# JuliaQuantumControl/QuOptimalControl.jl

Measured on AMD Instinct MI355X. Metric: GRAPE gradient-evals/sec, higher is better.
Workload: dtype f64; 1 GPU; C3: UnitaryGate 4x4, K=4, N=500 slices, ensemble E=1024 (one GPU, 1024 members/GPU), T=2.0; step = host->host grape_eval; parallelism=single GPU

## Files before the change

### quoptimalcontrol.jl_amd/csrc/grape_api.cpp

```cpp
#include "../../include/grape_hip.h"

#include <hip/hip_runtime.h>
#include <rccl/rccl.h>

#include <dlfcn.h>
#include <fcntl.h>
#include <time.h>
#include <unistd.h>

#include <algorithm>
#include <cmath>
#include <complex>
#include <cstdio>
#include <cstdlib>
#include <cstring>
#include <limits>
#include <atomic>
#include <condition_variable>
#include <mutex>
#include <thread>
#include <new>
#include <utility>
#include <string>
#include <vector>
// ... 104 lines not shown
    int32_t *d_any_sp_i = nullptr;
    double2 *d_any_sp_c = nullptr;
    size_t any_sp_i_bytes = 0, any_sp_c_bytes = 0, any_sp_nnz = 0, any_sp_ntouch = 0;
    bool ctrl_scaled = false;
    double *d_ctrl_scale = nullptr;
    size_t act_var_bytes = 0;
    double *d_act_bn = nullptr;
    double2 *d_act_bs = nullptr;
    int32_t *d_act_bo = nullptr;
    size_t states_bytes = 0;
    int tp_C = 0, tp_S = 0;
    double2 *d_tp_q = nullptr, *d_tp_r = nullptr, *d_tp_m = nullptr;
    double *d_tp_z = nullptr;
    double2 *d_tp_vec = nullptr;
    size_t tp_cap[6] = {0, 0, 0, 0, 0, 0};
    int tp_G = 0, tp_g = 0;
    double2 *d_tp_a = nullptr;
    bool direct_publish = true;
    bool pen_on = false;
    std::vector<double> pen_w;
    double *d_pen_w = nullptr;
    int rc_terms = 0;
    double2 *d_rc_R = nullptr;
    double *d_rc_rho = nullptr;
    double2 *d_rc_xs = nullptr;
    double *d_rc_rows = nullptr;
    size_t rc_xs_bytes = 0, rc_rows_bytes = 0;
    int rc_mode = 0;
    bool obs_on = false;
    int obs_n = 0, obs_per_member = 0;
    bool obs_want_y = false, obs_want_xf = false;
    double2 *d_obs_O = nullptr;
    double2 *d_obs_y = nullptr;
    double2 *d_obs_xf = nullptr;
    size_t obs_O_bytes = 0, obs_y_bytes = 0, obs_xf_bytes = 0;
    bool vjp_on = false;
    int vjp_n = 0, vjp_per_member = 0;
    bool vjp_has_y = false, vjp_has_x = false;
    double2 *d_vjp_O = nullptr;
    double2 *d_vjp_ybar = nullptr;
    double2 *d_vjp_xbar = nullptr;
    double *d_vjp_part = nullptr;
    double *d_vjp_g = nullptr;
    double *d_vjp_out = nullptr;
    size_t vjp_O_bytes = 0, vjp_ybar_bytes = 0, vjp_xbar_bytes = 0, vjp_part_bytes = 0, vjp_g_bytes = 0, vjp_out_bytes = 0;
    const double2 *obs_O_call = nullptr, *vjp_O_call = nullptr, *vjp_ybar_call = nullptr, *vjp_xbar_call = nullptr;
    double2 *obs_y_call = nullptr, *obs_xf_call = nullptr;
    double *vjp_G_call = nullptr;
    int obs_staged = 0, vjp_staged = 0;
    bool jvp_on = false;
    int jvp_n = 0, jvp_per_member = 0;
    bool jvp_has_y = false, jvp_has_x = false;
    double2 *d_jvp_O = nullptr;
    double *d_jvp_xdot = nullptr;
    double *d_jvp_xphys = nullptr;
    double2 *d_jvp_ydot = nullptr;
    double2 *d_jvp_xf = nullptr;
    size_t jvp_O_bytes = 0, jvp_xdot_bytes = 0, jvp_xphys_bytes = 0, jvp_ydot_bytes = 0, jvp_xf_bytes = 0;
    const double2 *jvp_O_call = nullptr;
    const double *jvp_xdot_call = nullptr;
    double2 *jvp_ydot_call = nullptr, *jvp_xf_call = nullptr;
    int jvp_ndir = 0, jvp_multi = 0;
    int lds_cap = 0;
    bool traj_valid = false;
    int traj_mode = 0;
    double2 *d_traj_w = nullptr;
    double *d_traj_x = nullptr;
    size_t traj_w_bytes = 0, traj_x_bytes = 0;
    int basis_M = 0;
    int basis_nb = 1;
    double *d_basis_phi = nullptr;
    double *d_basis_x0 = nullptr;
    bool bounds_on = false;
    double *d_bounds = nullptr;
    double *d_slope = nullptr;
    double risk_beta = 0.0;
    double *d_risk_rows = nullptr;
    double *d_risk_p = nullptr;
    size_t risk_rows_bytes = 0, risk_p_bytes = 0;
    int risk_slot = 0;
    bool risk_evaluated = false;
    std::vector<double> h_wts;
    bool pair_ah_env = true;
    bool mf_publish = true;
    unsigned long long seq = 0;
    std::string kernel_log;
    int x_upload = 1;
    double *d_x_bar = nullptr;
    hipStream_t stream = nullptr;
    bool ops_set = false, evaluated = false;
    bool unitary = false;
    bool herm_states = false;
    std::vector<hipEvent_t> ev;
    std::vector<char> ev_has_mid;
    std::vector<float> smp_total, smp_first;
    uint64_t ev_issued = 0, ev_folded = 0;
    uint64_t launches = 0;
    double ev_total_ms = 0.0;
    int64_t ev_count = 0;
    hipEvent_t ev_dev = nullptr;
    bool dev_pending = false;
    ncclComm_t comm = nullptr;
    int comm_rank = 0, comm_size = 1;
    bool is_group = false;
    std::vector<grape_ctx *> sub;
    std::vector<int> sub_lo;
    struct GroupWorker *worker = nullptr;
    double group_tm[5] = {0, 0, 0, 0, 0};
    uint64_t group_tm_n = 0;
    double timeout_s = 600.0;
    double eval_ema_s = 0.0;
    mutable std::string err;
};

static constexpr size_t kEventRing = 256;

static thread_local std::string *g_kernel_log = nullptr;
struct KernelLogScope {
    explicit KernelLogScope(std::string *log, bool append = false) { g_kernel_log = log; if (log && !append) log->clear(); }
    ~KernelLogScope() { g_kernel_log = nullptr; }
};
namespace grape {
void log_kernel(const char *expr)
{
    std::string *log = g_kernel_log;
    if (!log || !expr) return;
    while (*expr == '(' || *expr == ' ') ++expr;
    const char *end = expr;
    while (*end && *end != '<' && *end != ')' && *end != ' ') ++end;
    if (!log->empty()) log->push_back(';');
    log->append(expr, (size_t)(end - expr));
}
}

static thread_local std::string g_create_err = "";

static int fail(const grape_ctx *ctx, int code, const std::string &msg)
{
    if (ctx) ctx->err = msg; else g_create_err = msg;
    return code;
}

#define HIP_TRY(ctx, call)                                                                     \
    do {                                                                                       \
        hipError_t e__ = (call);                                                               \
        if (e__ != hipSuccess)                                                                 \
            return fail(ctx, e__ == hipErrorOutOfMemory ? GRAPE_ERR_ALLOC : GRAPE_ERR_HIP,     \
                        std::string(#call) + ": " + hipGetErrorString(e__));                   \
    } while (0)

static double now_s()
{
    timespec t;
    clock_gettime(CLOCK_MONOTONIC, &t);
    return (double)t.tv_sec + 1e-9 * (double)t.tv_nsec;
}

static const grape_ctx *lead_of(const grape_ctx *c) { return c->is_group ? c->sub[0] : c; }
static grape_ctx *lead_of(grape_ctx *c) { return c->is_group ? c->sub[0] : c; }

template <class T>
static int grow(grape_ctx *c, T **ptr, size_t *cap, size_t want, const char *who, const char *what)
{
    if (want <= *cap) return GRAPE_OK;
    (void)hipFree(*ptr);
    *ptr = nullptr;
// ... 433 lines not shown
    if (const char *ev = std::getenv("GRAPE_MPB")) {
        const int v = std::atoi(ev);
        if (c->family == 0 && v >= 1 && v * W <= wmax) c->MPB = v;
    }
    if (c->MPB > E) c->MPB = E;
    bool xg_in_lds = true;
    if (c->family == 0) {
        const size_t cap = 150 * 1024;
        auto lds_need = [&](int mpb, bool in_lds) {
            return c->pair ? grape::sweep_pair_lds_bytes(cfg->n, mpb, c->LT, S, cfg->n_controls, in_lds)
                           : grape::sweep_small_lds_bytes(cfg->n, mpb, c->LT, S, cfg->n_controls, in_lds);
        };
        while (c->MPB > 1 && lds_need(c->MPB, true) > cap)
            c->MPB /= 2;
        xg_in_lds = lds_need(c->MPB, true) <= cap;
    }
    c->NB = (E + c->MPB - 1) / c->MPB;
    c->ksplit = grape::reduce_ksplit(E);

    const size_t nn = (size_t)cfg->n * cfg->n, K = cfg->n_controls;
    const size_t Q = KN(c) + 1;
    c->ws_unit = c->family == 0 ? (size_t)S * nn * c->CH : (c->family == 1 ? (size_t)N * c->TSZ : (size_t)N * nn);
    const size_t ops_elems = c->family != 1 ? (size_t)E * (K + 3) * nn : (size_t)c->EU * (2 * K + 3) * c->TSZ;
    const bool exact = cfg->gradient == GRAPE_GRADIENT_EXACT;
    const bool keepl = (cfg->flags & GRAPE_FLAG_KEEP_COSTATES) != 0 || exact;
    {
        size_t free_b = 0, total_b = 0;
        if (hipMemGetInfo(&free_b, &total_b) != hipSuccess || free_b == 0) {
            hipDeviceProp_t pr{};
            free_b = hipGetDeviceProperties(&pr, c->device) == hipSuccess ? pr.totalGlobalMem : ~(size_t)0 >> 1;
        }
        const size_t rest = 2 * (sizeof(double2) * ops_elems + sizeof(double) * (size_t)E * Q * c->B) + ((size_t)64 << 20);
        c->ws_budget = free_b > rest ? (size_t)(0.9 * (double)(free_b - rest)) : 0;
        if (const char *ev = std::getenv("GRAPE_MAX_WORKSPACE_BYTES")) c->ws_budget = (size_t)std::strtoull(ev, nullptr, 10);
        if (const char *ev = std::getenv("GRAPE_TEST_FAIL_REPLAN")) c->test_fail_replan = std::atoi(ev);
        if (!plan_chunk(c, 1 + (keepl ? 1 : 0))) {
            const std::string msg = "grape_create: not even " + std::to_string(c->family == 0 ? c->MPB : 2) +
                                    " members' workspace fits the budget of " + std::to_string(c->ws_budget) + " bytes";
            delete c;
            return fail(nullptr, GRAPE_ERR_ALLOC, msg);
        }
    }

    auto alloc = [&](void **p, size_t bytes) -> hipError_t {
        c->bytes += bytes;
        return hipMalloc(p, bytes);
    };
    hipError_t e = hipSuccess;
    if (e == hipSuccess) e = alloc((void **)&c->d_ops, sizeof(double2) * ops_elems);
    if (e == hipSuccess) e = alloc((void **)&c->d_wts, sizeof(double) * E);
    const size_t Bn = (size_t)c->B;
    if (e == hipSuccess) e = alloc((void **)&c->d_x, sizeof(double) * KN(c) * Bn);
    if (e == hipSuccess) e = alloc((void **)&c->d_fg, sizeof(double) * Q * Bn);
    if (e == hipSuccess) e = alloc((void **)&c->d_props, sizeof(double2) * c->ws_elems * ws_batch(c));
    if (e == hipSuccess && keepl) e = alloc((void **)&c->d_costates, sizeof(double2) * c->ws_elems * ws_batch(c));
    if (e == hipSuccess && exact && c->family == 0) e = alloc((void **)&c->d_zphi, sizeof(double) * 2 * E * Bn);
    const bool want_rows = c->family != 0 || (cfg->flags & GRAPE_FLAG_MEMBER_RESULTS) || exact;
    if (e == hipSuccess && want_rows) e = alloc((void **)&c->d_member_out, sizeof(double) * E * Q * Bn);
    if (e == hipSuccess) e = alloc((void **)&c->d_partial, sizeof(double) * c->ksplit * Q);
    if (e == hipSuccess && c->family == 0) e = alloc((void **)&c->d_block_out, sizeof(double) * c->NB * Q * Bn);
    if (e == hipSuccess && c->family == 0 && !xg_in_lds)
        e = alloc((void **)&c->d_xg_scratch,
                  sizeof(double) * Bn * c->NB * ((size_t)c->MPB * c->CH * ((size_t)S * K + 1) + c->MPB));
    if (e == hipSuccess && (cfg->flags & GRAPE_FLAG_PHASE_STAMPS)) {
        const size_t sb = sizeof(unsigned long long) * Bn * E * W * grape::kStampSlots;
        e = alloc((void **)&c->d_stamps, sb);
        if (e == hipSuccess) e = hipMemset(c->d_stamps, 0, sb);
    }
    const unsigned hflags = hipHostMallocMapped | hipHostMallocCoherent | hipHostMallocPortable;
    if (e == hipSuccess) e = hipHostMalloc((void **)&c->h_stage, sizeof(double) * Q * Bn, hflags);
    if (e == hipSuccess) e = hipHostGetDevicePointer((void **)&c->d_h_stage, c->h_stage, 0);
    if (e == hipSuccess) e = hipHostMalloc((void **)&c->h_fg, sizeof(double) * Q * Bn, hflags);
    if (e == hipSuccess) e = hipHostGetDevicePointer((void **)&c->d_h_fg, c->h_fg, 0);
    if (e == hipSuccess) e = hipHostMalloc((void **)&c->h_flag, 64 + sizeof(unsigned long long) * grape::kMaxMflags, hflags);
    if (e == hipSuccess) e = hipHostGetDevicePointer((void **)&c->d_h_flag, c->h_flag, 0);
    if (e == hipSuccess) { std::memset(c->h_flag, 0, 64 + sizeof(unsigned long long) * grape::kMaxMflags); e = alloc((void **)&c->d_done_counter, 64); }
    if (e == hipSuccess) e = hipMemset(c->d_done_counter, 0, 64);
    {
        const char *dp = std::getenv("GRAPE_DIRECT_PUBLISH");
        c->direct_publish = !(dp && dp[0] == '0');
        c->mf_publish = !env_off("GRAPE_MF_PUBLISH");
        c->pair_ah_env = !env_off("GRAPE_PAIR_AH");
        c->pair_image_env = !env_off("GRAPE_PAIR_IMAGE");
    }
    {
        const char *xu = std::getenv("GRAPE_X_UPLOAD");
        int mode = 2;
        if (xu) mode = !std::strcmp(xu, "memcpy") ? 0 : (!std::strcmp(xu, "kernel") ? 1 : 2);
        int large_bar = 0;
        if (mode == 2 && e == hipSuccess &&
            (hipDeviceGetAttribute(&large_bar, hipDeviceAttributeIsLargeBar, dev) != hipSuccess || !large_bar))
            mode = 1;
        if (mode == 2 && e == hipSuccess) {
            void *p = nullptr;
            if (hipExtMallocWithFlags(&p, sizeof(double) * KN(c) * Bn, hipDeviceMallocFinegrained) == hipSuccess && p) {
                const int fd = open("/dev/zero", O_RDONLY);
                const bool ok = fd >= 0 && read(fd, p, 64) == 64;
                if (fd >= 0) close(fd);
                if (ok) {
                    c->d_x_bar = (double *)p;
                    c->bytes += sizeof(double) * KN(c) * Bn;
                } else {
                    (void)hipFree(p);
                    mode = 1;
                }
            } else {
                (void)hipGetLastError();
                mode = 1;
            }
        }
        c->x_upload = mode;
        if (std::getenv("GRAPE_DEBUG"))
            std::fprintf(stderr, "[grape] x upload mode %d (large_bar=%d)\n", mode, large_bar);
    }
    if (e == hipSuccess) e = hipStreamCreateWithFlags(&c->stream, hipStreamNonBlocking);
    if (e == hipSuccess) e = hipEventCreateWithFlags(&c->ev_dev, hipEventDisableTiming);
    if (e == hipSuccess) e = hipEventCreateWithFlags(&c->ev_done, hipEventDisableTiming);
    if (e == hipSuccess && (cfg->flags & GRAPE_FLAG_TIME_KERNELS)) {
        c->ev.reserve(3 * kEventRing);
        c->ev_has_mid.assign(kEventRing, 0);
        for (size_t i = 0; i < 3 * kEventRing && e == hipSuccess; ++i) {
            hipEvent_t evn = nullptr;
            e = hipEventCreate(&evn);
            if (e == hipSuccess) c->ev.push_back(evn);
        }
    }
    if (e != hipSuccess) {
        std::string msg = std::string("grape_create: device allocation failed: ") + hipGetErrorString(e);
        free_all(c);
        return fail(nullptr, e == hipErrorOutOfMemory ? GRAPE_ERR_ALLOC : GRAPE_ERR_HIP, msg);
    }
    *out = c;
    return GRAPE_OK;
}

static void shard_plan(int E, int G, std::vector<int> &lo)
{
    const int per = (E + G - 1) / G;
    lo.clear();
    for (int s = 0; s < E; s += per) lo.push_back(s);
    lo.push_back(E);
}

extern "C" int grape_create(const grape_config *cfg, grape_ctx **out)
{
    DeviceGuard guard;
    if (out) *out = nullptr;
    if (!cfg || !out) return fail(nullptr, GRAPE_ERR_INVALID_ARG, "grape_create: null argument");
    int rc = validate_config(cfg);
    if (rc) return rc;

    int ndev = 0;
    if (hipGetDeviceCount(&ndev) != hipSuccess || ndev < 1)
        return fail(nullptr, GRAPE_ERR_NO_DEVICE, "grape_create: no HIP device visible");
    const bool group = cfg->n_devices >= 2 || (cfg->flags & GRAPE_FLAG_FORCE_COLLECTIVE);
    std::vector<int> devs;
    if (cfg->n_devices >= 2) {
        for (int i = 0; i < cfg->n_devices; ++i) {
            const int d = cfg->device_ids[i];
            if (d < 0 || d >= ndev)
                return fail(nullptr, GRAPE_ERR_NO_DEVICE,
                            "grape_create: device_ids[" + std::to_string(i) + "]=" + std::to_string(d) +
                                " but " + std::to_string(ndev) + " HIP device(s) are visible");
            for (int j = 0; j < i; ++j)
                if (cfg->device_ids[j] == d && !(cfg->flags & GRAPE_FLAG_GROUP_PEER_SUM))
                    return fail(nullptr, GRAPE_ERR_INVALID_ARG, "grape_create: device_ids holds a duplicate "
// ... 292 lines not shown
        }
        c->pen_w = w;
        c->pen_on = on;
        return GRAPE_OK;
    }
    return shard_set_penalties(c, w, on);
}

static const char *why_running_cost_not_served(const grape_ctx *c, int mode)
{
    if (const char *why = why_exchange_not_served(c)) return why;
    if (c->family != 0) return "the operator dimension must be 2, 3 or 4 (the register-resident kernel family)";
    if (c->cfg.sys_type != GRAPE_UNITARY_GATE)
        return "StateTransfer / CoherenceTransfer (the sandwich needs a second term) are not served; hold the states as n x m columns under UnitaryGate";
    if (c->cfg.gradient == GRAPE_GRADIENT_EXACT) {
        if (mode != GRAPE_TRAJ_EXACT)
            return "gradient = exact is not served (the running cost's gradient is first order in dt; "
                   "grape_set_running_cost_derivative(GRAPE_TRAJ_EXACT) makes it exact)";
        return nullptr;
    }
    if (c->cfg.objective != GRAPE_OBJECTIVE_FOM) return "objective = c1 is not served";
    return nullptr;
}

extern "C" int grape_set_running_cost(grape_ctx *c, int32_t n_terms, const double *R, const double *rho)
{
    DeviceGuard guard;
    if (!c) return fail(nullptr, GRAPE_ERR_INVALID_ARG, "grape_set_running_cost: null context");
    c->traj_valid = false;
    const bool off = n_terms == 0 || !R;
    if (!off) {
        if (n_terms < 0 || n_terms > 4)
            return fail(c, GRAPE_ERR_INVALID_ARG, "grape_set_running_cost: n_terms = " + std::to_string(n_terms) + " (must be in 0..4)");
        if (!rho) return fail(c, GRAPE_ERR_INVALID_ARG, "grape_set_running_cost: null rho");
        const char *why = why_running_cost_not_served(c, c->rc_mode);
        if (!why && c->risk_beta != 0.0)
            why = "a risk is set: grape_set_risk does not serve a running cost (the members' J_k are not in the member rows)";
        if (why) return fail(c, GRAPE_ERR_UNSUPPORTED, std::string("grape_set_running_cost: ") + why);
        const size_t nr = 2 * (size_t)c->cfg.n * c->m * c->cfg.n_ensemble * n_terms, nw = (size_t)c->cfg.n_slices * n_terms;
        if (int rc = check_finite(c, R, nr, "grape_set_running_cost", "R", 2)) return rc;
        if (int rc = check_finite(c, rho, nw, "grape_set_running_cost", "rho")) return rc;
    }
    if (c->is_group) {
        c->rc_terms = 0;
        return GRAPE_OK;
    }
    if (int rc = drain(c, c)) return rc;
    void *d_R = nullptr, *d_rho = nullptr;
    if (!off) {
        const size_t rb = sizeof(double2) * (size_t)c->cfg.n * c->m * c->cfg.n_ensemble * n_terms;
        const size_t wb = sizeof(double) * (size_t)c->cfg.n_slices * n_terms;
        if (int rc = device_copies(c, "grape_set_running_cost", R, rb, &d_R, rho, wb, &d_rho)) return rc;
    }
    (void)hipFree(c->d_rc_R);
    (void)hipFree(c->d_rc_rho);
    c->d_rc_R = (double2 *)d_R;
    c->d_rc_rho = (double *)d_rho;
    c->rc_terms = off ? 0 : n_terms;
    return GRAPE_OK;
}

extern "C" int grape_set_running_cost_derivative(grape_ctx *c, int32_t mode)
{
    DeviceGuard guard;
    if (!c) return fail(nullptr, GRAPE_ERR_INVALID_ARG, "grape_set_running_cost_derivative: null context");
    c->traj_valid = false;
    if (mode != GRAPE_TRAJ_FIRST_ORDER && mode != GRAPE_TRAJ_EXACT)
        return fail(c, GRAPE_ERR_INVALID_ARG, "grape_set_running_cost_derivative: mode = " + std::to_string(mode) +
                                              " (must be GRAPE_TRAJ_FIRST_ORDER = 0 or GRAPE_TRAJ_EXACT = 1)");
    if (mode == GRAPE_TRAJ_EXACT) {
        if (const char *why = why_running_cost_not_served(c, mode))
            return fail(c, GRAPE_ERR_UNSUPPORTED, std::string("grape_set_running_cost_derivative: ") + why);
    } else if (c->rc_terms > 0 && c->cfg.gradient == GRAPE_GRADIENT_EXACT) {
        return fail(c, GRAPE_ERR_UNSUPPORTED, "grape_set_running_cost_derivative: a running cost is set on a gradient = exact context "
                                              "(it takes the exact mode only; switch the running cost off first)");
    }
    if (c->is_group) return GRAPE_OK;
    if (int rc = drain(c, c)) return rc;
    c->rc_mode = mode;
    return GRAPE_OK;
}

static int wait_stream(grape_ctx *c, hipStream_t stream);

static int risk_check_weights(const grape_ctx *c, const double *wts, const char *who)
{
    double W = 0.0;
    for (int k = 0; k < c->cfg.n_ensemble; ++k) {
        if (!(wts[k] >= 0.0) || !std::isfinite(wts[k]))
            return fail(c, GRAPE_ERR_INVALID_ARG, std::string(who) + ": weight[" + std::to_string(k) + "] = " + std::to_string(wts[k]) +
                                                      " (a risk needs finite ensemble weights >= 0)");
        W += wts[k];
    }
    if (!(W > 0.0))
        return fail(c, GRAPE_ERR_INVALID_ARG, std::string(who) + ": the ensemble weights sum to 0 (a risk needs a positive sum)");
    return GRAPE_OK;
}

extern "C" int grape_set_risk(grape_ctx *c, double beta)
{
    DeviceGuard guard;
    if (!c) return fail(nullptr, GRAPE_ERR_INVALID_ARG, "grape_set_risk: null context");
    c->traj_valid = false;
    if (!std::isfinite(beta))
        return fail(c, GRAPE_ERR_INVALID_ARG, "grape_set_risk: beta = " + std::to_string(beta) + " (must be finite; 0 switches the risk off)");
    if (beta != 0.0) {
        const char *why = why_exchange_not_served(c);
        if (!why && c->rc_terms > 0) why = "a running cost is in force (the members' J_k are not in the member rows)";
        if (why) return fail(c, GRAPE_ERR_UNSUPPORTED, std::string("grape_set_risk: ") + why);
        if (c->ops_set)
            if (int rc = risk_check_weights(c, c->h_wts.data(), "grape_set_risk")) return rc;
    }
    if (c->is_group) return GRAPE_OK;
    if (int rc = drain(c, c)) return rc;
    c->risk_beta = beta;
    c->risk_evaluated = false;
    return GRAPE_OK;
}

extern "C" int grape_get_risk_weights(grape_ctx *c, double *p)
{
    DeviceGuard guard;
    if (!c) return fail(nullptr, GRAPE_ERR_INVALID_ARG, "grape_get_risk_weights: null context");
    if (!p) return fail(c, GRAPE_ERR_INVALID_ARG, "grape_get_risk_weights: p is null");
    if (c->risk_beta == 0.0 || !c->risk_evaluated || !c->d_risk_p)
        return fail(c, GRAPE_ERR_NOT_READY, "grape_get_risk_weights: no evaluation with a risk in force yet");
    if (int rc = drain(c, c)) return rc;
    HIP_TRY(c, hipMemcpy(p, c->d_risk_p, sizeof(double) * (size_t)c->cfg.n_ensemble, hipMemcpyDeviceToHost));
    return GRAPE_OK;
}

extern "C" int grape_set_basis(grape_ctx *c, int32_t n_params, int32_t n_bases, const double *phi, const double *x0)
{
    DeviceGuard guard;
    if (!c) return fail(nullptr, GRAPE_ERR_INVALID_ARG, "grape_set_basis: null context");
    c->traj_valid = false;
    const int K = c->cfg.n_controls, N = c->cfg.n_slices;
    const bool off = !phi || n_params == 0;
    if (!off) {
        if (n_params < 1 || n_params > N)
            return fail(c, GRAPE_ERR_INVALID_ARG, "grape_set_basis: n_params = " + std::to_string(n_params) + " (must be in 1..n_slices)");
        if (n_bases != 1 && n_bases != K)
            return fail(c, GRAPE_ERR_INVALID_ARG, "grape_set_basis: n_bases = " + std::to_string(n_bases) + " (must be 1 or n_controls)");
        if (int rc = check_finite(c, phi, (size_t)N * n_params * n_bases, "grape_set_basis", "phi")) return rc;
        if (int rc = check_finite(c, x0, x0 ? KN(c) : 0, "grape_set_basis", "x0")) return rc;
    }
    if (int rc = drain(c, lead_of(c))) return rc;
    void *d_phi = nullptr, *d_x0 = nullptr;
    if (!off) {
        const size_t np = (size_t)N * n_params * n_bases;
        if (int rc = device_copies(c, "grape_set_basis", phi, sizeof(double) * np, &d_phi, x0, x0 ? sizeof(double) * KN(c) : 0, &d_x0))
            return rc;
    }
    (void)hipFree(c->d_basis_phi);
    (void)hipFree(c->d_basis_x0);
    c->d_basis_phi = (double *)d_phi;
    c->d_basis_x0 = (double *)d_x0;
    c->basis_M = off ? 0 : n_params;
    c->basis_nb = off ? 1 : n_bases;
    return GRAPE_OK;
}

extern "C" int grape_set_bounds(grape_ctx *c, const double *lo, const double *hi)
{
    DeviceGuard guard;
    if (!c) return fail(nullptr, GRAPE_ERR_INVALID_ARG, "grape_set_bounds: null context");
    c->traj_valid = false;
    const int K = c->cfg.n_controls;
    if (!lo != !hi) return fail(c, GRAPE_ERR_INVALID_ARG, "grape_set_bounds: lo and hi must both be given, or both be null");
    bool on = false;
    for (int k = 0; lo && k < K; ++k) {
        const bool free_k = lo[k] == -INFINITY && hi[k] == INFINITY;
        if (!free_k && !(std::isfinite(lo[k]) && std::isfinite(hi[k]) && lo[k] < hi[k]))
            return fail(c, GRAPE_ERR_INVALID_ARG, "grape_set_bounds: control " + std::to_string(k) + ": need finite lo < hi, or lo = -inf and hi = +inf");
        on = on || !free_k;
    }
    if (int rc = drain(c, lead_of(c))) return rc;
    if (on) {
        void *d_b = nullptr, *d_s = nullptr;
        std::vector<double> lh(2 * (size_t)K);
        std::copy(lo, lo + K, lh.begin());
        std::copy(hi, hi + K, lh.begin() + K);
        if (int rc = device_copies(c, "grape_set_bounds", lh.data(), sizeof(double) * 2 * K, &d_b, nullptr,
                                   c->d_slope ? 0 : sizeof(double) * KN(c) * (size_t)c->B, &d_s))
            return rc;
        (void)hipFree(c->d_bounds);
        c->d_bounds = (double *)d_b;
        if (d_s) c->d_slope = (double *)d_s;
    }
    c->bounds_on = on;
    return GRAPE_OK;
}

static grape::BasisOp basis_op(const grape_ctx *c, bool project, int n_x)
{
    grape::BasisOp op;
    op.project = project ? 1 : 0;
    op.phi = c->d_basis_phi;
    op.x0 = c->d_basis_x0;
    op.K = c->cfg.n_controls;
    op.N = c->cfg.n_slices;
    op.M = c->basis_M;
    op.n_bases = c->basis_nb;
    op.n_x = n_x;
    if (c->bounds_on) {
        op.bounded = 1;
        op.lo = c->d_bounds;
        op.hi = c->d_bounds + c->cfg.n_controls;
        op.slope = c->d_slope;
    }
    return op;
}

extern "C" int grape_get_controls(grape_ctx *c, const double *theta, double *x)
{
    DeviceGuard guard;
    if (!c) return GRAPE_ERR_INVALID_ARG;
    c->traj_valid = false;
    if (!theta || !x) return fail(c, GRAPE_ERR_INVALID_ARG, "grape_get_controls: null argument");
    if (!pulse_map(c)) {
        std::memmove(x, theta, sizeof(double) * KN(c));
        return GRAPE_OK;
    }
    grape_ctx *lead = lead_of(c);
    HIP_TRY(c, hipSetDevice(lead->device));
    if (int rc = order_behind_device_call(c, lead)) return rc;
    std::memcpy(lead->h_stage, theta, sizeof(double) * KP(c));
    const grape::BasisOp op = basis_op(c, false, 1);
    grape::DoneSignal d;
    d.basis = &op;
    HIP_TRY(c, grape::launch_copy(lead->d_h_stage, lead->d_x, (int)KN(c), lead->stream, d));
    HIP_TRY(c, hipMemcpyAsync(lead->h_fg, lead->d_x, sizeof(double) * KN(c), hipMemcpyDeviceToHost, lead->stream));
    const int rc = wait_stream(lead, lead->stream);
    if (rc) return c->is_group ? fail(c, rc, lead->err) : rc;
    std::memcpy(x, lead->h_fg, sizeof(double) * KN(c));
    return GRAPE_OK;
}

static long act_min_units(const grape_ctx *c)
{
    if (const char *e = std::getenv("GRAPE_ACTION_MIN")) return std::atol(e);
    if (c->NT == 2) return 3L * c->compute_units / 8;
    return c->NT == 1 && !c->pack2 ? 15L * c->compute_units / 16 : 9L * c->compute_units / 8;
}

extern "C" int grape_set_operators(grape_ctx *c, const double *A, const double *B, const double *Xi,
                                   const double *Xt, const double *wts)
{
    if (!c) return GRAPE_ERR_INVALID_ARG;
    c->traj_valid = false;
    if (!A || !B || !Xi || !Xt || !wts)
        return fail(c, GRAPE_ERR_INVALID_ARG, "grape_set_operators: null argument");
    if (c->is_group) {
        const size_t nn2 = 2 * (size_t)c->cfg.n * c->cfg.n, Kc = c->cfg.n_controls;
        const size_t nm2 = 2 * (size_t)c->cfg.n * (c->cfg.n_state_cols ? c->cfg.n_state_cols : c->cfg.n);
        for (size_t i = 0; i < c->sub.size(); ++i) {
            const size_t lo = (size_t)c->sub_lo[i];
            const int rc = grape_set_operators(c->sub[i], A + lo * nn2, B + lo * Kc * nn2, Xi + lo * nm2,
                                               Xt + lo * nm2, wts + lo);
            if (rc) {
                c->ops_set = false;
                return fail(c, rc, c->sub[i]->err);
            }
        }
        c->ops_set = true;
        c->evaluated = false;
        return GRAPE_OK;
    }
    if (c->risk_beta != 0.0)
        if (int rc = risk_check_weights(c, wts, "grape_set_operators")) return rc;
    c->ops_set = false;
    DeviceGuard guard;
    if (int rc = drain(c, c)) return rc;
    const char *who = "grape_set_operators";
    const size_t nn = (size_t)c->cfg.n * c->cfg.n, K = c->cfg.n_controls, E = c->cfg.n_ensemble;
    std::vector<double> xi_pad, xt_pad;
    if (c->m != c->cfg.n) {
        const size_t nm = (size_t)c->cfg.n * c->m;
        try {
            xi_pad.assign(2 * E * nn, 0.0);
            xt_pad.assign(2 * E * nn, 0.0);
        } catch (...) {
            return fail(c, GRAPE_ERR_ALLOC, "grape_set_operators: out of host memory");
        }
        for (size_t k = 0; k < E; ++k) {
            std::memcpy(xi_pad.data() + 2 * k * nn, Xi + 2 * k * nm, sizeof(double) * 2 * nm);
            std::memcpy(xt_pad.data() + 2 * k * nn, Xt + 2 * k * nm, sizeof(double) * 2 * nm);
        }
        Xi = xi_pad.data();
        Xt = xt_pad.data();
    }
    std::vector<double> packed;
    try {
        packed.assign(c->family != 1 ? 2 * E * (K + 3) * nn : 2 * (size_t)c->EU * (2 * K + 3) * c->TSZ, 0.0);
    } catch (...) {
        return fail(c, GRAPE_ERR_ALLOC, "grape_set_operators: out of host memory");
    }
    if (c->family == 0) {
        const double dt = c->cfg.duration / c->cfg.n_slices;
        auto scaled = [&](double *dst, const double *src, size_t count) {
            for (size_t e = 0; e < count; ++e) {
                dst[2 * e] = dt * src[2 * e + 1];
                dst[2 * e + 1] = -dt * src[2 * e];
            }
        };
        for (size_t k = 0; k < E; ++k) {
            double *dst = packed.data() + 2 * k * (K + 3) * nn;
            scaled(dst, A + 2 * k * nn, nn);
            scaled(dst + 2 * nn, B + 2 * k * K * nn, K * nn);
// ... 484 lines not shown
                    c->states_bytes = 0;
                    if (keep) { (void)hipFree(c->d_costates); c->d_costates = nullptr; c->bytes -= old_b; }
                    c->ws_invalid = true;
                    c->ws_keep_costates = keep;
                    c->ops_set = false;
                }
                if (c->test_fail_replan > 0) {
                    --c->test_fail_replan;
                    return fail(c, GRAPE_ERR_ALLOC, "grape_set_operators: workspace allocation failed (GRAPE_TEST_FAIL_REPLAN)");
                }
                HIP_TRY(c, hipMalloc((void **)&c->d_props, new_b));
                c->bytes += new_b;
                if (keep && !c->d_costates) { HIP_TRY(c, hipMalloc((void **)&c->d_costates, new_b)); c->bytes += new_b; }
                c->ws_invalid = false;
            }
        }
        if (chunked(c) && (c->tp_C || c->thin_dpp))
            return fail(c, GRAPE_ERR_ALLOC, "grape_set_operators: a chunked time axis on a member-chunked workspace (budget too small for this ensemble)");
    }
    if (c->family == 2) {
        c->any_blocks = grape::any_prop_blocks(c->cfg.n, c->cfg.n_slices, (long)c->cfg.n_ensemble * c->B, c->compute_units);
        const size_t per_block = sizeof(double2) * 6 * nn * (size_t)c->Ec * ws_batch(c);
        const size_t cap = std::min<size_t>((size_t)8 << 30, std::max<size_t>(c->ws_budget / 4, per_block));
        while (c->any_blocks > 1 && per_block * (size_t)c->any_blocks > cap)
            c->any_blocks = (c->any_blocks + 1) / 2;
        c->tp_C = c->tp_S = 0;
        {
            const long units = (long)c->cfg.n_ensemble * c->B, N = c->cfg.n_slices;
            if (c->cfg.n >= 17 && N >= 16 && 2 * units <= (long)c->compute_units && !env_on("GRAPE_NO_TP") && !chunked(c) && !may_chunk(c)) {
                const long s_lat = std::max(4L, std::lround(std::sqrt((double)N / 2.0)));
                long C = std::min((long)c->compute_units / units, (N + s_lat - 1) / s_lat);
                if (const char *e = std::getenv("GRAPE_TP_CHUNKS")) C = std::atol(e);
                if (C > N / 2) C = N / 2;
                while (C >= 2 && (per_block + sizeof(double2) * 3 * nn * (size_t)c->Ec * ws_batch(c)) * (size_t)C > cap)
                    C = (C + 1) / 2;
                if (C >= 2) {
                    c->tp_S = (int)((N + C - 1) / C);
                    c->tp_C = (int)((N + c->tp_S - 1) / c->tp_S);
                }
            }
        }
        if (c->tp_C) {
            const size_t bytes = sizeof(double2) * nn * (size_t)c->cfg.n_ensemble * c->B * (size_t)c->tp_C;
            const char *what = "the time chunks' products";
            if (int rc = grow(c, &c->d_tp_q, &c->tp_cap[0], bytes, who, what)) return rc;
            if (int rc = grow(c, &c->d_tp_r, &c->tp_cap[1], bytes, who, what)) return rc;
            if (int rc = grow(c, &c->d_tp_m, &c->tp_cap[2], bytes, who, what)) return rc;
        }
        const size_t need = per_block * (size_t)std::max(c->any_blocks, std::max(1, c->tp_C));
        if (int rc = grow(c, &c->d_scratch, &c->scratch_bytes, need, who, "the propagator blocks' scratch matrices")) return rc;
    }
    if (thin) {
        c->unitary = false;
        if (!c->d_vecs) {
            c->bytes += sizeof(double) * E * 4 * VS;
            HIP_TRY(c, hipMalloc((void **)&c->d_vecs, sizeof(double) * E * 4 * VS));
        }
        HIP_TRY(c, hipMemcpy(c->d_vecs, vecs.data(), sizeof(double) * E * 4 * VS, hipMemcpyHostToDevice));
        const size_t rec = sizeof(double2) * (size_t)c->Ec * ((size_t)c->cfg.n_slices + 1) * VS * ws_batch(c);
        if (int rc = grow(c, &c->d_states, &c->states_bytes, rec, who, "the forward states")) return rc;
    } else if (!herm || c->exact_w1) {
        if (int rc = grow(c, &c->d_states, &c->states_bytes, sizeof(double2) * c->ws_elems * ws_batch(c), who, "the forward states")) return rc;
    }
    HIP_TRY(c, hipMemcpy(c->d_ops, packed.data(), sizeof(double) * packed.size(), hipMemcpyHostToDevice));
    if (c->family == 0 && c->pair && c->pair_image_env) {
        const size_t ib = sizeof(double2) * (size_t)grape::pair_image_d2(c->cfg.n, c->cfg.n_controls) * E;
        if (!c->d_pair_img) {
            c->bytes += ib;
            HIP_TRY(c, hipMalloc((void **)&c->d_pair_img, ib));
        }
        SweepParams ip{};
        ip.ops = c->d_ops;
        ip.pair_img = c->d_pair_img;
        ip.img_only = 1;
        ip.K = c->cfg.n_controls;
        ip.E = c->cfg.n_ensemble;
        HIP_TRY(c, grape::launch_sweep_pair(c->cfg.n, 0, 0, ip, nullptr));
        HIP_TRY(c, hipStreamSynchronize(nullptr));
    }
    HIP_TRY(c, hipMemcpy(c->d_wts, wts, sizeof(double) * E, hipMemcpyHostToDevice));
    c->h_wts.assign(wts, wts + E);
    c->ops_set = true;
    c->evaluated = false;
    c->risk_evaluated = false;
    return GRAPE_OK;
}

static TileParams tile_params(const grape_ctx *c, const double *d_x, int n_x = 1)
{
    TileParams p{};
    p.n_x = n_x;
    p.ops = c->d_ops;
    p.x = d_x;
    p.props = c->d_props;
    p.states = c->d_states;
    p.costates = c->d_costates;
    p.member_out = c->d_member_out;
    p.K = c->cfg.n_controls;
    p.N = c->cfg.n_slices;
    p.E = c->EU;
    p.E_plan = c->EU;
    p.E_members = c->cfg.n_ensemble;
    p.pack2 = c->pack2 ? 1 : 0;
    p.n = c->cfg.n;
    p.s_forced = c->cfg.expm_squarings;
    p.variant = c->cfg.variant;
    p.dt = c->cfg.duration / c->cfg.n_slices;
    p.unitary = c->unitary ? 1 : 0;
    p.herm_states = c->herm_states ? 1 : 0;
    p.thin = c->thin ? (c->thin_dpp ? 2 : 1) : 0;
    p.herm_ctrl = c->herm_ctrl ? 1 : 0;
    p.vecs = c->d_vecs;
    p.cus = c->compute_units;
    p.tp_chunks = c->tp_C;
    p.tp_S = c->tp_S;
    p.tp_q = c->d_tp_q;
    p.tp_r = c->d_tp_r;
    p.tp_m = c->d_tp_m;
    p.tp_z = c->d_tp_z;
    p.tp_vec = c->d_tp_vec;
    p.tp_groups = c->tp_C ? c->tp_G : 0;
    p.tp_gsize = c->tp_g;
    p.tp_a = c->d_tp_a;
    if (c->tp_C && ((!c->unitary && !c->thin) || c->thin_dpp || c->grid)) {
        const size_t half = (size_t)c->EU * c->B * c->tp_C * c->NT * c->NT * 256;
        p.tp_qt = c->d_tp_q + half;
        p.tp_u = c->d_tp_r + half;
    }
    p.sparse = c->sparse_ctrl ? 1 : 0;
    p.sp_nz = c->sp_nz;
    p.sp_coef = c->d_sp_coef;
    p.sp_addr = c->d_sp_addr;
    p.hoist = c->hoist;
    p.ha = c->d_ha;
    p.ha_norm = c->d_ha_norm;
    p.gc = c->d_gc;
    p.gcn = c->d_gcn;
    p.action = c->action ? 1 : 0;
    if (c->action) {
        p.E = c->cfg.n_ensemble;
        p.E_plan = c->cfg.n_ensemble;
        p.pack2 = 0;
    }
    p.act_a = c->d_act_a;
    p.act_an = c->d_act_an;
    p.act_b = c->d_act_b;
    p.act_bf = c->d_act_bf;
    p.act_g = c->d_act_g ? c->d_act_g + 3 * (size_t)(c->cfg.n <= 16 ? 256 : 1024) : nullptr;
    p.act_gn = c->d_act_gn;
    p.act_R = (c->action || c->thin_dpp) ? c->act_R : 0;
    p.wrec = c->thin_dpp ? c->d_wrec : c->d_props;
    p.props_t = c->d_props_t;
    p.act_shared = c->act_shared ? 1 : 0;
    p.ctrl_scale = c->ctrl_scaled ? c->d_ctrl_scale : nullptr;
    p.ops_ref = c->d_ops;
    p.act_b_ref = c->d_act_b;
    p.act_bn = c->d_act_bn;
    p.act_bs = c->d_act_bs;
    p.act_bo = c->d_act_bo;
    return p;
}

static bool states_stored(const grape_ctx *c)
{
    if (c->exact_w1) return false;
    if (c->d_costates) return true;
    if (c->family == 2) return true;
    if (c->family == 0 || c->unitary || c->thin) return false;
    if (c->grid && !c->thin) return true;
    return !grape::tile_chain_is_split(tile_params(c, nullptr), false);
}

static bool pen_active(const grape_ctx *c) { return c->pen_on && c->comm_rank == 0; }

static grape::DoneSignal with_pen(const grape_ctx *c, grape::DoneSignal d, const double *d_x)
{
    if (pen_active(c)) {
        d.pen_x = d_x;
        d.pen_w = c->d_pen_w;
        d.pen_K = c->cfg.n_controls;
        d.pen_N = c->cfg.n_slices;
    }
    return d;
}

static grape::DoneSignal host_signal(grape_ctx *s, double *host_out)
{
    grape::DoneSignal d;
    d.counter = s->d_done_counter;
    d.flag = s->d_h_flag;
    d.seq = ++s->seq;
    d.host_out = host_out;
    return d;
}

static SweepParams sweep_params(const grape_ctx *c, const double *d_x, int n_x)
{
    SweepParams p{};
    p.ops = c->d_ops;
    p.pair_img = c->d_pair_img;
    p.x = d_x;
    p.wts = c->d_wts;
    p.MPB = c->MPB;
    p.BPX = c->NB;
    p.n_x = n_x;
    p.sk_magic = (uint32_t)((1ull << 32) / ((uint64_t)c->S * c->cfg.n_controls)) + 1u;
    p.K = c->cfg.n_controls;
    p.N = c->cfg.n_slices;
    p.E = c->cfg.n_ensemble;
    p.S = c->S;
    p.LT = c->LT;
    p.s_forced = c->cfg.expm_squarings;
    p.variant = c->cfg.variant;
    p.dt = c->cfg.duration / c->cfg.n_slices;
    return p;
}

static bool pair_antiherm(const grape_ctx *c)
{
    return c->family == 0 && c->pair && c->unitary && c->cfg.n == 4 && c->cfg.sys_type == GRAPE_UNITARY_GATE && !c->exact_w1 &&
           c->cfg.gradient != GRAPE_GRADIENT_EXACT && c->pair_ah_env;
}

static hipError_t launch_small_family(const grape_ctx *c, int sandwich, int mode, const SweepParams &p, hipStream_t stream)
{
    return c->pair ? grape::launch_sweep_pair(c->cfg.n, sandwich, mode, p, stream)
                   : grape::launch_sweep_small(c->cfg.n, sandwich, mode, p, stream);
}

static int upload_x(grape_ctx *s, int n_x, const double **d_x)
{
    const size_t kn = KN(s);
    *d_x = s->d_x;
    if (s->x_upload == 2)
        *d_x = s->d_x_bar;
    else if (s->x_upload == 1)
        HIP_TRY(s, grape::launch_copy(s->d_h_stage, s->d_x, (int)(kn * n_x), s->stream));
    else
        HIP_TRY(s, hipMemcpyAsync(s->d_x, s->h_stage, sizeof(double) * kn * n_x, hipMemcpyHostToDevice, s->stream));
    return GRAPE_OK;
}

static int group_allreduce(grape_ctx *g, size_t count, double *out0, hipStream_t st0)
{
    NCCL_TRY(g, g_rccl.GroupStart());
    for (size_t i = 0; i < g->sub.size(); ++i) {
        grape_ctx *s = g->sub[i];
        const ncclResult_t r = g_rccl.AllReduce(s->d_fg, i == 0 ? out0 : s->d_fg, count, ncclDouble, ncclSum, s->comm, i == 0 ? st0 : s->stream);
        if (r != ncclSuccess) {
            (void)g_rccl.GroupEnd();
            return fail(g, GRAPE_ERR_COMM, std::string("ncclAllReduce: ") + g_rccl.GetErrorString(r));
        }
    }
    NCCL_TRY(g, g_rccl.GroupEnd());
    return GRAPE_OK;
}

static void copy_out_rows(const double *h_fg, int n_x, size_t len, double *F, double *G)
{
    for (int b = 0; b < n_x; ++b) {
        if (G) std::memcpy(G + (size_t)b * len, h_fg + (size_t)b * (len + 1), sizeof(double) * len);
        if (F) F[b] = h_fg[(size_t)b * (len + 1) + len];
    }
}

static int rc_ensure(grape_ctx *c)
{
    const size_t nrows = c->cfg.gradient == GRAPE_GRADIENT_EXACT ? (size_t)c->cfg.n_ensemble : (size_t)c->Ec * ws_batch(c);
    const size_t rows = sizeof(double) * nrows * (KN(c) + 1);
    const size_t xs = c->unitary ? 0 : sizeof(double2) * (size_t)c->Ec * ws_batch(c) * c->S * c->CH * c->cfg.n * c->m;
    if (int rc = grow(c, &c->d_rc_rows, &c->rc_rows_bytes, rows, "grape_set_running_cost", "the members' running-cost rows")) return rc;
    if (int rc = grow(c, &c->d_rc_xs, &c->rc_xs_bytes, xs, "grape_set_running_cost", "the stored states of the general flow")) return rc;
    if (c->rc_terms > 0 && c->rc_mode == GRAPE_TRAJ_EXACT) {
        const size_t w = sizeof(double2) * (size_t)c->Ec * ws_batch(c) * c->S * c->CH * c->cfg.n * c->cfg.n;
        return grow(c, &c->d_traj_w, &c->traj_w_bytes, w, "grape_set_running_cost_derivative", "the exact derivative's per-slice blocks");
    }
    return GRAPE_OK;
}

static int risk_ensure(grape_ctx *c)
{
    const size_t E = (size_t)c->cfg.n_ensemble, B = (size_t)c->B;
    if (c->family == 0 && !c->d_member_out)
        if (int rc = grow(c, &c->d_risk_rows, &c->risk_rows_bytes, sizeof(double) * E * (KN(c) + 1) * B, "grape_set_risk", "the members' rows")) return rc;
    return grow(c, &c->d_risk_p, &c->risk_p_bytes, sizeof(double) * (E + 1) * B, "grape_set_risk", "the risk weights");
}

static grape::DoneSignal with_risk(const grape_ctx *c, grape::DoneSignal d, int slot)
{
    if (c->risk_beta != 0.0) {
        d.risk_beta = c->risk_beta;
        d.risk_p = c->d_risk_p + (size_t)slot * c->cfg.n_ensemble;
        d.risk_F = c->d_risk_p + (size_t)c->B * c->cfg.n_ensemble + slot;
    }
    return d;
}

// ... 122 lines not shown
        HIP_TRY(c, grape::launch_copy(c->jvp_xdot_call + (size_t)dir * KP(c), c->d_jvp_xphys + (size_t)dir * KN(c), (int)KN(c), stream, d));
    return GRAPE_OK;
}

static int enqueue_eval(grape_ctx *c, const double *d_x, double *d_fg, hipStream_t stream, int n_x = 1,
                        grape::DoneSignal done = grape::DoneSignal())
{
    if ((c->cfg.gradient == GRAPE_GRADIENT_EXACT || n_x > c->ws_B) && n_x > 1) {
        const size_t Qs = KN(c) + 1;
        for (int b = 0; b < n_x; ++b) {
            grape::DoneSignal db;
            if (b == n_x - 1 && done.flag) {
                db = done;
                db.stage_base = d_fg;
                db.n_total = (int)(Qs * n_x);
                db.mflags = nullptr;
            }
            c->risk_slot = b;
            const int rc = enqueue_eval(c, d_x + (size_t)b * KN(c), d_fg + (size_t)b * Qs, stream, 1, db);
            c->risk_slot = 0;
            if (rc) return rc;
        }
        return GRAPE_OK;
    }
    c->traj_valid = false;
    const bool risk = c->risk_beta != 0.0;
    if (risk) {
        const int rc = risk_ensure(c);
        if (rc) return rc;
    }
    double *const rows = c->d_member_out ? c->d_member_out : (risk ? c->d_risk_rows : nullptr);
    const bool rc_on = c->rc_terms > 0 && c->family == 0;
    if (rc_on) {
        const int rc = rc_ensure(c);
        if (rc) return rc;
    }
    if (c->vjp_on) {
        const int rc = rc_ensure(c);
        if (rc) return rc;
    }
    const bool keep_x = traj_exact(c) && c->family == 0 && (c->obs_on || c->vjp_on || c->jvp_on);
    if (keep_x) {
        const int rc = traj_exact_ensure(c, "grape_set_trajectory_derivative");
        if (rc) return rc;
    }
    KernelLogScope log_scope(&c->kernel_log);
    if (keep_x) HIP_TRY(c, grape::launch_copy(d_x, c->d_traj_x, (int)KN(c), stream));
    if (c->jvp_on && pulse_map(c)) {
        const int rc = jvp_tangent_map(c, stream);
        if (rc) return rc;
    }
    c->mf_wait = 0;
    SweepParams p = sweep_params(c, d_x, n_x);
    p.props = c->d_props;
    p.states = c->d_states;
    p.costates = c->d_costates;
    p.member_out = rows;
    p.block_out = c->d_block_out;
    p.stamps = c->d_stamps;
    p.xg_scratch = c->d_xg_scratch;
    p.dump_w1 = c->exact_w1 ? 1 : 0;
    p.zphi = c->d_zphi;
    p.vec = (c->family == 0 && c->pair && c->cfg.n == 4 && c->m == 1 && c->cfg.sys_type == GRAPE_UNITARY_GATE &&
             c->cfg.gradient != GRAPE_GRADIENT_EXACT && !env_off("GRAPE_PAIR_VEC")) ? 1 : 0;
    bool timed = (c->cfg.flags & GRAPE_FLAG_TIME_KERNELS) != 0;
    if (timed && (c->cfg.flags & GRAPE_FLAG_TIME_SAMPLED) && (c->launches++ & 7) != 0)
        timed = false;
    hipEvent_t e0 = nullptr, e1 = nullptr, emid = nullptr;
    if (timed) {
        if (c->ev_issued - c->ev_folded == kEventRing) {
            int rc = fold_events(c, 1);
            if (rc) return rc;
        }
        const size_t slot = (size_t)(c->ev_issued % kEventRing);
        e0 = c->ev[3 * slot];
        e1 = c->ev[3 * slot + 2];
        if (c->family == 1 || (c->family == 2 && c->any_blocks > 1)) emid = c->ev[3 * slot + 1];
        c->ev_has_mid[slot] = emid ? 1 : 0;
        c->ev_issued += 1;
        HIP_TRY(c, hipEventRecord(e0, stream));
    }
    const bool exact = c->cfg.gradient == GRAPE_GRADIENT_EXACT;
    if (exact) p.member_out = nullptr;
    const bool direct = c->family == 0 && c->NB == 1 && n_x == 1 && !exact && c->direct_publish && !done.probe_out &&
                        !done.stage_base && !pen_active(c) && !rc_on && !risk;
    const bool fold = !done.stage_base && tile_folds_reduce(c, n_x);
    if (direct) {
        p.direct_dst = done.flag && done.host_out ? done.host_out : d_fg;
        p.direct_flag = done.flag;
        p.direct_seq = done.seq;
    }
    const size_t nn = (size_t)c->cfg.n * c->cfg.n, Kc = (size_t)c->cfg.n_controls, Qrow = KN(c) + 1;
    auto launch_members = [&](int lo, int cnt) -> int {
        if (c->family == 0) {
            SweepParams q = p;
            q.ops = p.ops + (size_t)lo * (Kc + 3) * nn;
            if (p.pair_img) q.pair_img = p.pair_img + (size_t)lo * grape::pair_image_d2(c->cfg.n, (int)Kc);
            q.wts = p.wts + lo;
            if (p.member_out) q.member_out = p.member_out + (size_t)lo * Qrow;
            q.block_out = p.block_out + (size_t)(lo / c->MPB) * Qrow;
            if (p.zphi) q.zphi = p.zphi + 2 * (size_t)lo;
            q.E = cnt;
            q.BPX = (cnt + c->MPB - 1) / c->MPB;
            const int mode = c->unitary ? 2 : (c->d_costates ? 1 : 0), sand = c->cfg.sys_type != GRAPE_UNITARY_GATE;
            HIP_TRY(c, launch_small_family(c, sand, (mode == 2 && pair_antiherm(c)) ? 3 : mode, q, stream));
            if (rc_on) {
                SweepParams r = q;
                r.rc_only = 1;
                r.rc_terms = c->rc_terms;
                r.rc_m = c->m;
                r.rc_unitary = c->unitary ? 1 : 0;
                r.rc_CH = c->CH;
                r.rc_Etot = c->cfg.n_ensemble;
                r.rc_R = c->d_rc_R + (size_t)lo * c->cfg.n * c->m;
                r.rc_rho = c->d_rc_rho;
                r.rc_xs = c->d_rc_xs;
                r.rc_rows = c->d_rc_rows;
                if (c->rc_mode == GRAPE_TRAJ_EXACT) {
                    r.rc_exact = 1;
                    r.traj_w = c->d_traj_w;
                    if (exact) {
                        r.rc_unweighted = 1;
                        r.rc_rows = c->d_rc_rows + (size_t)lo * Qrow;
                    }
                }
                HIP_TRY(c, launch_small_family(c, 0, mode, r, stream));
            }
            if (c->obs_on) {
                SweepParams o = q;
                o.obs_only = 1;
                o.obs_n = c->obs_want_y ? c->obs_n : 0;
                o.obs_m = c->m;
                o.obs_per_member = c->obs_per_member;
                o.obs_CH = c->CH;
                o.obs_Etot = c->cfg.n_ensemble;
                o.obs_E0 = lo;
                o.obs_O = c->obs_O_call;
                o.obs_y = c->obs_want_y ? c->obs_y_call : nullptr;
                o.obs_xf = c->obs_want_xf ? c->obs_xf_call : nullptr;
                o.obs_staged = c->obs_want_y ? c->obs_staged : 0;
                HIP_TRY(c, launch_small_family(c, sand, mode, o, stream));
            }
            if (c->vjp_on) {
                SweepParams v = vjp_params(c, q, lo);
                HIP_TRY(c, launch_small_family(c, 0, mode, v, stream));
                if (lo + cnt == c->cfg.n_ensemble) {
                    v.vjp_only = 2;
                    HIP_TRY(c, launch_small_family(c, 0, mode, v, stream));
                }
            }
            if (c->jvp_on) {
                SweepParams v = jvp_params(c, q, lo);
                HIP_TRY(c, launch_small_family(c, 0, mode, v, stream));
            }
            if (exact) {
                grape::ExactParams xq{};
                xq.ops = q.ops;
                xq.x = d_x;
                xq.props = c->d_props;
                xq.states = c->d_states;
                xq.costates = c->d_costates;
                xq.member_out = c->d_member_out + (size_t)lo * Qrow;
                xq.K = c->cfg.n_controls;
                xq.N = c->cfg.n_slices;
                xq.E = cnt;
                xq.S = c->S;
// ... 138 lines not shown
    KernelLogScope log_scope(&c->kernel_log, true);
    grape::IpcParams ip{};
    ip.own_row = row;
    ip.Q = (int)((KN(c) + 1) * (size_t)n_x);
    ip.Qpad = (int)(((KN(c) + 1) * (size_t)c->B + 255) / 256 * 256);
    ip.rank = c->comm_rank;
    ip.n_ranks = c->ipc_ranks;
    ip.parity = (int)(c->ipc_evals & 1);
    ip.target = (unsigned long long)c->ipc_ranks * (c->ipc_count[ip.parity] + 1);
    for (int j = 0; j < c->ipc_ranks; ++j) ip.mbox[j] = c->ipc_mbox[j];
    const double lim = std::min(120.0, std::max(5.0, c->timeout_s));
    ip.spin_limit = (long long)(lim * 1e6);
    ip.out = out;
    ip.done = done;
    ip.fail_word = c->d_h_flag + 1;
    if (grape::launch_ipc_allreduce(ip, stream) != hipSuccess)
        return fail(c, GRAPE_ERR_HIP, "ipc_allreduce_kernel: launch failed");
    c->ipc_evals += 1;
    c->ipc_count[ip.parity] += 1;
    return GRAPE_OK;
}

static int ipc_check(grape_ctx *c)
{
    if (c->broken)
        return fail(c, GRAPE_ERR_COMM, "the context is unusable: an earlier multi-device evaluation failed part-way (see the error it returned)");
    if (c->ipc_ranks > 1 && c->h_flag) {
        __atomic_thread_fence(__ATOMIC_ACQUIRE);
        if (((volatile unsigned long long *)c->h_flag)[1] != 0) {
            c->broken = true;
            return fail(c, GRAPE_ERR_COMM, "a mailbox exchange issued through the device-pointer path gave up (a peer is gone or stuck): "
                                           "its [G, F] were poisoned with NaN; the context is unusable");
        }
    }
    return GRAPE_OK;
}

static int wait_stream(grape_ctx *c, hipStream_t stream)
{
    const double t0 = now_s();
    long nap_ns = 20000;
    for (unsigned it = 0;; ++it) {
        const hipError_t q = hipStreamQuery(stream);
        if (q == hipSuccess) return GRAPE_OK;
        if (q != hipErrorNotReady) HIP_TRY(c, q);
        if ((it & 63) != 63) continue;
        const double el = now_s() - t0;
        if (el < 500e-6) continue;
        if (el > c->timeout_s)
            return fail(c, GRAPE_ERR_TIMEOUT, "evaluation did not finish within " + std::to_string(c->timeout_s) +
                                                  " s (GRAPE_EVAL_TIMEOUT_S): device presumed hung");
        timespec nap{0, nap_ns};
        nanosleep(&nap, nullptr);
        if (nap_ns < 1000000) nap_ns *= 2;
    }
}

static void shard_stage_x(grape_ctx *s, const double *x, int n_x)
{
    const size_t kn = KN(s);
    if (s->x_upload == 2) {
        std::memcpy(s->d_x_bar, x, sizeof(double) * kn * n_x);
        __atomic_thread_fence(__ATOMIC_SEQ_CST);
#if defined(__x86_64__)
        __builtin_ia32_sfence();
#endif
    } else {
        std::memcpy(s->h_stage, x, sizeof(double) * kn * n_x);
    }
}

static int shard_issue(grape_ctx *s, int n_x, double *target, bool signal)
{
    HIP_TRY(s, hipSetDevice(s->device));
    if (int rc = order_behind_device_call(s, s)) return rc;
    const double *d_x = nullptr;
    if (int rc = upload_x(s, n_x, &d_x)) return rc;
    grape::DoneSignal done;
    if (signal) {
        done = host_signal(s, target);
        if (s->mf_publish) done.mflags = s->d_h_flag + 8;
        target = s->d_fg;
    }
    return enqueue_eval(s, d_x, target, s->stream, n_x, done);
}

static int shard_enqueue_host(grape_ctx *s, const double *x, int n_x, double *target, bool signal)
{
    shard_stage_x(s, x, n_x);
    return shard_issue(s, n_x, target, signal);
}

static int shard_issue_group(grape_ctx *s)
{
    int rc = shard_issue(s, s->group ? s->group->group_nx : 1, s->d_fg, false);
    if (rc == GRAPE_OK && s->ev_done && hipEventRecord(s->ev_done, s->stream) != hipSuccess)
        rc = fail(s, GRAPE_ERR_HIP, "hipEventRecord failed");
    return rc;
}

static int shard_launch_arrive(grape_ctx *s)
{
    KernelLogScope log_scope(&s->kernel_log, true);
    grape_ctx *g = s->group;
    grape::ArriveParams ap{};
    ap.rows.n = (int)g->sub.size();
    for (size_t i = 0; i < g->sub.size(); ++i) ap.rows.p[i] = g->sub[i]->d_fg;
    ap.Q = (int)((KN(g) + 1) * (size_t)g->group_nx);
    ap.arrive = g->d_arrive;
    ap.finished = g->d_arrive + ((KN(g) + 1) * (size_t)g->B + 255) / 256;
    ap.out = nullptr;
    ap.done = g->group_done;
    if (grape::launch_shard_arrive(ap, s->stream) != hipSuccess)
        return fail(s, GRAPE_ERR_HIP, "shard_arrive_kernel: launch failed");
    return GRAPE_OK;
}
static int shard_issue_group_arrive(grape_ctx *s)
{
    int rc = shard_issue(s, s->group->group_nx, s->d_fg, false);
    if (rc == GRAPE_OK) rc = shard_launch_arrive(s);
    return rc;
}

void GroupWorker::run()
{
    (void)hipSetDevice(shard->device);
    uint64_t seen = 0;
    double idle_since = now_s();
    for (;;) {
        unsigned spins = 0;
        while (req.load(std::memory_order_acquire) == seen) {
            if (stop.load(std::memory_order_relaxed)) return;
#if defined(__x86_64__)
            __builtin_ia32_pause();
#endif
            if ((++spins & 4095) == 0) {
                if (now_s() - idle_since > 2e-3) {
                    std::unique_lock<std::mutex> lk(mu);
                    asleep.store(true, std::memory_order_seq_cst);
                    cv.wait(lk, [&] { return req.load(std::memory_order_seq_cst) != seen || stop.load(); });
                    asleep.store(false, std::memory_order_seq_cst);
                }
            }
        }
        seen = req.load(std::memory_order_acquire);
        rc = job ? job(shard) : 0;
        done.store(seen, std::memory_order_release);
        idle_since = now_s();
    }
}

static int wait_flag(grape_ctx *s)
{
    volatile unsigned long long *flag = s->h_flag;
    const unsigned long long want = s->seq;
    const int mf = s->mf_wait;
    auto all_flags = [&]() {
        for (int i = 0; i < mf; ++i)
            if (flag[8 + i] != want) return false;
        return true;
    };
    const double t0 = now_s();
    bool napped = false;
    auto done = [&](double el, bool first_look) {
        __atomic_thread_fence(__ATOMIC_ACQUIRE);
        if (napped && first_look)
            s->eval_ema_s *= 0.5;
// ... 745 lines not shown
                                            "holds one block of members only");
    if (reuse && !was_valid)
        return fail(c, GRAPE_ERR_NOT_READY, std::string(who) + ": d_x is null (reuse), but the workspace does not hold the trajectory of a "
                                            "device form: another call has evaluated, changed a setting or failed since");
    hipStream_t st = (hipStream_t)stream;
    rc = traj_device_prologue(c);
    if (rc) return rc;
    if (pulse_map(c)) {
        rc = grow(c, &c->d_jvp_xphys, &c->jvp_xphys_bytes, sizeof(double) * KN(c) * (multi ? (size_t)n_dir : 1), who,
                  "the direction of the physical pulse");
        if (rc) return rc;
        rc = grow(c, &c->d_vjp_out, &c->vjp_out_bytes, sizeof(double) * (KP(c) + 1), who, "the projected row");
        if (rc) return rc;
    }
    if (multi && traj_exact(c)) {
        rc = traj_exact_ensure(c, who, jvp_exact_images(c));
        if (rc) return rc;
    }
    const bool want_y = d_ydot != nullptr && n_obs > 0;
    c->jvp_n = n_obs;
    c->jvp_per_member = per_member;
    c->jvp_has_y = want_y;
    c->jvp_has_x = d_Xdot_final != nullptr;
    c->jvp_O_call = (const double2 *)d_O;
    c->jvp_xdot_call = d_xdot;
    c->jvp_ydot_call = (double2 *)d_ydot;
    c->jvp_xf_call = (double2 *)d_Xdot_final;
    if (!reuse) {
        c->jvp_on = true;
        rc = traj_device_eval(c, d_x, pulse_map(c) ? c->d_vjp_out : c->d_fg, st);
        c->jvp_on = false;
        if (rc) return rc;
    } else {
        if (traj_exact(c)) {
            rc = traj_exact_ensure(c, who, jvp_exact_images(c));
            if (rc) return rc;
        }
        KernelLogScope log_scope(&c->kernel_log);
        if (pulse_map(c)) {
            rc = jvp_tangent_map(c, st);
            if (rc) return rc;
        }
        SweepParams q = sweep_params(c, nullptr, 1);
        q.props = c->d_props;
        const SweepParams v = jvp_params(c, q, 0);
        const int mode = c->unitary ? 2 : (c->d_costates ? 1 : 0);
        HIP_TRY(c, launch_small_family(c, 0, mode, v, st));
    }
    HIP_TRY(c, hipEventRecord(c->ev_dev, st));
    c->dev_pending = true;
    c->traj_valid = !chunked(c);
    return GRAPE_OK;
}

extern "C" int grape_eval_jvp_device(grape_ctx *c, const double *d_x, const double *d_xdot, int32_t n_obs, int32_t per_member,
                                     const double *d_O, double *d_ydot, double *d_Xdot_final, void *stream)
{
    DeviceGuard guard;
    if (!c) return fail(nullptr, GRAPE_ERR_INVALID_ARG, "grape_eval_jvp_device: null context");
    return eval_jvp_device(c, "grape_eval_jvp_device", false, d_x, 0, d_xdot, n_obs, per_member, d_O, d_ydot, d_Xdot_final, stream);
}

extern "C" int grape_eval_jvp_multi_device(grape_ctx *c, const double *d_x, int32_t n_dir, const double *d_xdot, int32_t n_obs,
                                           int32_t per_member, const double *d_O, double *d_ydot, double *d_Xdot_final,
                                           void *stream)
{
    DeviceGuard guard;
    if (!c) return fail(nullptr, GRAPE_ERR_INVALID_ARG, "grape_eval_jvp_multi_device: null context");
    return eval_jvp_device(c, "grape_eval_jvp_multi_device", true, d_x, n_dir, d_xdot, n_obs, per_member, d_O, d_ydot, d_Xdot_final,
                           stream);
}

static bool fom_fast(const grape_ctx *c) { return !c->is_group && !c->comm && c->ipc_ranks <= 1 && c->family == 0 && c->rc_terms == 0 && c->risk_beta == 0.0; }

static int fom_issue(grape_ctx *c, const double *x, int n_x)
{
    const size_t kn = KN(c);
    HIP_TRY(c, hipSetDevice(c->device));
    if (!c->d_fom_member) {
        HIP_TRY(c, hipMalloc((void **)&c->d_fom_member, sizeof(double) * (size_t)c->cfg.n_ensemble * c->B));
        HIP_TRY(c, hipMalloc((void **)&c->d_fom_rows, sizeof(double) * (size_t)c->NB * c->B));
    }
    const bool param = pulse_map(c);
    if (param)
        std::memcpy(c->h_stage, x, sizeof(double) * KP(c) * n_x);
    else
        shard_stage_x(c, x, n_x);
    if (int rc = order_behind_device_call(c, c)) return rc;
    KernelLogScope log_scope(&c->kernel_log);
    const double *d_x = c->d_x;
    const grape::BasisOp bop = basis_op(c, false, n_x);
    if (param) {
        grape::DoneSignal bd;
        bd.basis = &bop;
        HIP_TRY(c, grape::launch_copy(c->d_h_stage, c->d_x, (int)(kn * n_x), c->stream, bd));
    } else {
        if (int rc = upload_x(c, n_x, &d_x)) return rc;
        c->kernel_log.clear();
    }
    grape::DoneSignal done = host_signal(c, c->d_h_fg);
    c->mf_wait = 0;
    SweepParams p = sweep_params(c, d_x, n_x);
    p.fom_only = 1;
    p.fom_objective = c->cfg.objective;
    p.fom_member = c->d_fom_member;
    p.fom_rows = c->d_fom_rows;
    const bool direct = c->NB == 1 && n_x == 1 && c->direct_publish && !pen_active(c);
    if (direct) {
        p.direct_dst = done.host_out;
        p.direct_flag = done.flag;
        p.direct_seq = done.seq;
    }
    HIP_TRY(c, launch_small_family(c, c->cfg.sys_type != GRAPE_UNITARY_GATE, c->unitary ? 2 : 0, p, c->stream));
    if (direct)
        return GRAPE_OK;
    if (!pen_active(c)) {
        if (c->mf_publish) {
            done.mflags = c->d_h_flag + 8;
            c->mf_wait = grape::reduce_rows_mflags(1, n_x);
        }
        HIP_TRY(c, grape::launch_reduce_rows(c->d_fom_rows, c->d_fg, c->NB, 1, n_x, c->stream, done));
        return GRAPE_OK;
    }
    for (int b = 0; b < n_x; ++b) {
        grape::DoneSignal db;
        if (b == n_x - 1) {
            db = done;
            db.stage_base = c->d_fg;
            db.n_total = n_x;
        }
        HIP_TRY(c, grape::launch_reduce_rows(c->d_fom_rows + (size_t)b * c->NB, c->d_fg + b, c->NB, 1, 1, c->stream,
                                             with_pen(c, db, d_x + (size_t)b * kn)));
    }
    return GRAPE_OK;
}

extern "C" int grape_eval_fom(grape_ctx *c, int32_t n_x, const double *x, double *F, double *member_F)
{
    DeviceGuard guard;
    if (!c) return GRAPE_ERR_INVALID_ARG;
    c->traj_valid = false;
    if (!x || !F) return fail(c, GRAPE_ERR_INVALID_ARG, "grape_eval_fom: x or F is null");
    if (n_x < 1 || n_x > c->B)
        return fail(c, GRAPE_ERR_INVALID_ARG, "grape_eval_fom: n_x must be in 1..max(1, grape_config.max_batch)");
    if (!c->ops_set) return fail(c, GRAPE_ERR_NOT_READY, "grape_eval_fom: operators not set");
    const size_t kn = KP(c), E = (size_t)c->cfg.n_ensemble;
    if (!fom_fast(c)) {
        if (!member_F)
            return eval_host(c, n_x, x, F, nullptr, "grape_eval_fom");
        const bool risk = c->risk_beta != 0.0;
        for (grape_ctx *s : c->is_group ? c->sub : std::vector<grape_ctx *>{c})
            if (!s->d_member_out && !risk)
                return fail(c, GRAPE_ERR_NOT_READY, "grape_eval_fom: member_F needs a context created with GRAPE_FLAG_MEMBER_RESULTS");
        for (int b = 0; b < n_x; ++b) {
            int rc = eval_host(c, 1, x + (size_t)b * kn, F + b, nullptr, "grape_eval_fom");
            if (rc) return rc;
            if (risk && !c->d_member_out) {
                rc = wait_stream(c, c->stream);
                if (rc) return rc;
                const size_t Q = KN(c) + 1;
                HIP_TRY(c, hipMemcpy2D(member_F + (size_t)b * E, sizeof(double), c->d_risk_rows + (Q - 1), sizeof(double) * Q,
                                       sizeof(double), E, hipMemcpyDeviceToHost));
                continue;
            }
            rc = grape_get_member_results(c, member_F + (size_t)b * E, nullptr);
            if (rc) return rc;
// ... 561 lines not shown
    }
    return GRAPE_OK;
}

extern "C" int grape_get_member_results(grape_ctx *c, double *foms, double *grads)
{
    DeviceGuard guard;
    if (!c) return GRAPE_ERR_INVALID_ARG;
    if (!c->evaluated) return fail(c, GRAPE_ERR_NOT_READY, "grape_get_member_results: no evaluation yet");
    if (c->is_group) {
        const size_t kn = KN(c);
        for (size_t i = 0; i < c->sub.size(); ++i) {
            const size_t lo = (size_t)c->sub_lo[i];
            const int rc = grape_get_member_results(c->sub[i], foms ? foms + lo : nullptr, grads ? grads + lo * kn : nullptr);
            if (rc) return group_fail(c, c->sub[i], rc);
        }
        return GRAPE_OK;
    }
    if (!c->d_member_out)
        return fail(c, GRAPE_ERR_NOT_READY, "grape_get_member_results: create the context with GRAPE_FLAG_MEMBER_RESULTS");
    HIP_TRY(c, hipSetDevice(c->device));
    HIP_TRY(c, hipDeviceSynchronize());
    const size_t kn = KN(c), Q = kn + 1, E = c->cfg.n_ensemble;
    std::vector<double> h(E * Q);
    HIP_TRY(c, hipMemcpy(h.data(), c->d_member_out, sizeof(double) * E * Q, hipMemcpyDeviceToHost));
    for (size_t k = 0; k < E; ++k) {
        if (foms) foms[k] = h[k * Q + kn];
        if (grads) std::memcpy(grads + k * kn, h.data() + k * Q, sizeof(double) * kn);
    }
    return GRAPE_OK;
}

static int fetch_slab(grape_ctx *c, const double2 *d_ws, int member, cplx *out, bool odd_transposed = false)
{
    if (c->family == 1) {
        const size_t N = c->cfg.n_slices, TSZ = c->TSZ;
        const int n = c->cfg.n, NT = c->NT;
        const int unit = c->pack2 ? member / 2 : member, off = c->pack2 ? 8 * (member & 1) : 0;
        std::vector<cplx> h(N * TSZ);
        HIP_TRY(c, hipMemcpy(h.data(), d_ws + (size_t)unit * N * TSZ, sizeof(cplx) * h.size(),
                             hipMemcpyDeviceToHost));
        for (size_t t = 0; t < N; ++t)
            for (int I = 0; I < NT; ++I)
                for (int J = 0; J < NT; ++J)
                    for (int r = 0; r < 4; ++r)
                        for (int l = 0; l < 64; ++l) {
                            int row = 16 * I + 4 * r + (l >> 4) - off, col = 16 * J + (l & 15) - off;
                            if (odd_transposed && (t & 1)) std::swap(row, col);
                            if (row >= 0 && col >= 0 && row < n && col < n)
                                out[t * n * n + row + (size_t)n * col] =
                                    h[t * TSZ + (size_t)((I * NT + J) * 4 + r) * 64 + l];
                        }
        return GRAPE_OK;
    }
    if (c->family == 2) {
        const size_t nn2 = (size_t)c->cfg.n * c->cfg.n, N2 = c->cfg.n_slices;
        HIP_TRY(c, hipMemcpy(out, d_ws + (size_t)member * N2 * nn2, sizeof(cplx) * N2 * nn2, hipMemcpyDeviceToHost));
        return GRAPE_OK;
    }
    const size_t nn = (size_t)c->cfg.n * c->cfg.n, S = c->S, LT = c->CH, N = c->cfg.n_slices;
    std::vector<cplx> h(S * nn * LT);
    HIP_TRY(c, hipMemcpy(h.data(), d_ws + (size_t)member * S * nn * LT, sizeof(cplx) * h.size(),
                         hipMemcpyDeviceToHost));
    for (size_t t = 0; t < N; ++t) {
        const size_t L = t / S, j = t % S;
        for (size_t e = 0; e < nn; ++e)
            out[t * nn + e] = h[(j * nn + e) * LT + L];
    }
    return GRAPE_OK;
}

extern "C" int grape_get_trajectory(grape_ctx *c, int32_t member, double *props, double *states,
                                    double *costates)
{
    DeviceGuard guard;
    if (!c) return GRAPE_ERR_INVALID_ARG;
    if (!c->evaluated) return fail(c, GRAPE_ERR_NOT_READY, "grape_get_trajectory: no evaluation yet");
    if (member < 0 || member >= c->cfg.n_ensemble)
        return fail(c, GRAPE_ERR_INVALID_ARG, "grape_get_trajectory: member out of range");
    if (c->is_group) {
        int local = 0;
        grape_ctx *s = owner_of(c, member, &local);
        const int rc = grape_get_trajectory(s, local, props, states, costates);
        return rc ? group_fail(c, s, rc) : GRAPE_OK;
    }
    if (chunked(c))
        return fail(c, GRAPE_ERR_NOT_READY,
                    "grape_get_trajectory: the workspace of this context holds " + std::to_string(c->Ec) + " of its " +
                    std::to_string(c->cfg.n_ensemble) + " members at a time (grape_info.member_chunk): no stored trajectory to return");
    if ((costates && !c->d_costates) || ((costates || states) && c->exact_w1))
        return fail(c, GRAPE_ERR_NOT_READY,
                    "grape_get_trajectory: costates need GRAPE_FLAG_KEEP_COSTATES at grape_create (this exact-gradient flow "
                    "stores neither states nor costates)");
    if (props && c->action)
        return fail(c, GRAPE_ERR_NOT_READY,
                    "grape_get_trajectory: this flow applies exp(G_t) to vectors and forms no propagators; create the "
                    "context with GRAPE_FLAG_KEEP_COSTATES");
    if (states && !states_stored(c))
        return fail(c, GRAPE_ERR_NOT_READY,
                    "grape_get_trajectory: forward states are stored only by the debug flow; create the "
                    "context with GRAPE_FLAG_KEEP_COSTATES");
    HIP_TRY(c, hipSetDevice(c->device));
    HIP_TRY(c, hipDeviceSynchronize());
    const int n = c->cfg.n;
    const size_t nn = (size_t)n * n, N = c->cfg.n_slices, K = c->cfg.n_controls;
    std::vector<cplx> P(N * nn);
    int rc = fetch_slab(c, c->d_props, member, P.data(), c->thin && !c->thin_dpp && !c->grid);
    if (rc) return rc;
    if (props) std::memcpy(props, P.data(), sizeof(cplx) * N * nn);
    std::vector<cplx> xs_full, ls_full;
    double *states_user = states, *costates_user = costates;
    if (c->m != n) {
        if (states) { xs_full.resize((N + 1) * nn); states = reinterpret_cast<double *>(xs_full.data()); }
        if (costates) { ls_full.resize((N + 1) * nn); costates = reinterpret_cast<double *>(ls_full.data()); }
    }
    auto narrow = [&](const std::vector<cplx> &full, double *user) {
        const size_t nm = (size_t)n * c->m;
        for (size_t t = 0; t <= N; ++t)
            std::memcpy(reinterpret_cast<cplx *>(user) + t * nm, full.data() + t * nn, sizeof(cplx) * nm);
    };
    if (states) {
        cplx *X = reinterpret_cast<cplx *>(states);
        rc = fetch_slab(c, c->d_states, member, X);
        if (rc) return rc;
        const cplx *Pl = P.data() + (N - 1) * nn, *Xl = X + (N - 1) * nn;
        cplx *Xn = X + N * nn;
        std::vector<cplx> tmp(nn);
        const bool sand = c->cfg.sys_type != GRAPE_UNITARY_GATE;
        for (int j = 0; j < n; ++j)
            for (int i = 0; i < n; ++i) {
                cplx s = 0.0;
                for (int k = 0; k < n; ++k)
                    s += sand ? Xl[i + k * n] * std::conj(Pl[j + k * n]) : Pl[i + k * n] * Xl[k + j * n];
                (sand ? tmp[i + j * n] : Xn[i + j * n]) = s;
            }
        if (sand)
            for (int j = 0; j < n; ++j)
                for (int i = 0; i < n; ++i) {
                    cplx s = 0.0;
                    for (int k = 0; k < n; ++k) s += Pl[i + k * n] * tmp[k + j * n];
                    Xn[i + j * n] = s;
                }
    }
    if (costates) {
        cplx *Lc = reinterpret_cast<cplx *>(costates);
        rc = fetch_slab(c, c->d_costates, member, Lc);
        if (rc) return rc;
        if (c->family != 1) {
            HIP_TRY(c, hipMemcpy(Lc + N * nn, c->d_ops + (size_t)member * (K + 3) * nn + (K + 2) * nn,
                                 sizeof(cplx) * nn, hipMemcpyDeviceToHost));
        } else {
            std::vector<cplx> h(c->TSZ);
            const int unit = c->pack2 ? member / 2 : member, off = c->pack2 ? 8 * (member & 1) : 0;
            HIP_TRY(c, hipMemcpy(h.data(), c->d_ops + ((size_t)unit * (2 * K + 3) + 2 * K + 2) * c->TSZ,
                                 sizeof(cplx) * c->TSZ, hipMemcpyDeviceToHost));
            for (int I = 0; I < c->NT; ++I)
                for (int J = 0; J < c->NT; ++J)
                    for (int r = 0; r < 4; ++r)
                        for (int l = 0; l < 64; ++l) {
                            const int row = 16 * I + 4 * r + (l >> 4) - off, col = 16 * J + (l & 15) - off;
                            if (row >= 0 && col >= 0 && row < n && col < n)
                                Lc[N * nn + row + (size_t)n * col] = h[(size_t)((I * c->NT + J) * 4 + r) * 64 + l];
                        }
        }
    }
    if (c->m != n) {
        if (states_user) narrow(xs_full, states_user);
        if (costates_user) narrow(ls_full, costates_user);
    }
    return GRAPE_OK;
}

extern "C" int grape_get_kernel_time(grape_ctx *c, double *total_ms, int64_t *launches, int32_t reset)
{
    DeviceGuard guard;
    if (!c) return GRAPE_ERR_INVALID_ARG;
    if (c->is_group) {
        double worst = 0.0;
        int64_t n = 0;
        for (grape_ctx *s : c->sub) {
            double ms = 0.0;
            int64_t cnt = 0;
            const int rc = grape_get_kernel_time(s, &ms, &cnt, reset);
            if (rc) return group_fail(c, s, rc);
            if (ms > worst) worst = ms;
            n = cnt;
// ... 117 lines not shown
```

### quoptimalcontrol.jl_amd/csrc/grape_kernels.hpp

```cpp
#pragma once
#include <hip/hip_runtime.h>
#include <stddef.h>
#include <stdint.h>
#include <type_traits>

namespace grape {

void log_kernel(const char *expr);
#define GRAPE_LAUNCH(KERNEL, ...)                        \
    do {                                                 \
        ::grape::log_kernel(#KERNEL);                    \
        hipLaunchKernelGGL(KERNEL, __VA_ARGS__);         \
    } while (0)
#define GRAPE_LAUNCH_AS(NAME, KERNEL, ...)               \
    do {                                                 \
        ::grape::log_kernel(NAME);                       \
        hipLaunchKernelGGL(KERNEL, __VA_ARGS__);         \
    } while (0)


constexpr double kTheta8 = 0.08;

struct BasisOp {
    int32_t project = 0;
// ... 41 lines not shown
    double *block_out;
    unsigned long long *stamps;
    double *xg_scratch;
    int32_t K, N, E;
    int32_t S;
    int32_t LT;
    int32_t MPB;
    int32_t BPX;
    int32_t n_x;
    uint32_t sk_magic;
    int32_t s_forced;
    int32_t variant;
    int32_t plast_lds;
    double dt;
    double *direct_dst;
    unsigned long long *direct_flag;
    unsigned long long direct_seq;
    int32_t dump_w1;
    double *zphi;
    int32_t tune;
    int32_t vec;
    double *fom_member;
    double *fom_rows;
    int32_t fom_only;
    int32_t fom_objective;
    int32_t rc_only;
    int32_t rc_terms;
    int32_t rc_m;
    int32_t rc_unitary;
    int32_t rc_CH;
    int32_t rc_Etot;
    const double2 *rc_R;
    const double *rc_rho;
    double2 *rc_xs;
    double *rc_rows;
    int32_t obs_only;
    int32_t obs_n;
    int32_t obs_m;
    int32_t obs_per_member;
    int32_t obs_CH;
    int32_t obs_Etot;
    int32_t obs_E0;
    const double2 *obs_O;
    double2 *obs_y;
    double2 *obs_xf;
    int32_t vjp_only;
    int32_t vjp_n;
    int32_t vjp_m;
    int32_t vjp_per_member;
    int32_t vjp_unitary;
    int32_t vjp_CH;
    int32_t vjp_Etot;
    int32_t vjp_E0;
    const double2 *vjp_O;
    const double2 *vjp_ybar;
    const double2 *vjp_xbar;
    double2 *vjp_xs;
    double *vjp_rows;
    double *vjp_part;
    double *vjp_G;
    int32_t obs_staged;
    int32_t vjp_staged;
    int32_t jvp_only;
    int32_t jvp_n;
    int32_t jvp_m;
    int32_t jvp_per_member;
    int32_t jvp_CH;
    int32_t jvp_Etot;
    int32_t jvp_E0;
    const double2 *jvp_O;
    const double *jvp_xdot;
    double2 *jvp_ydot;
    double2 *jvp_xf;
    int32_t traj_exact;
    double2 *traj_w;
    const double *traj_x;
    int32_t rc_exact;
    int32_t rc_unweighted;
    int32_t jvp_ndir;
    int32_t jvp_multi;
    int64_t jvp_dir_xdot, jvp_dir_ydot, jvp_dir_xf, jvp_dir_w;
    double2 *pair_img;
    int32_t img_only;
};
constexpr int kParityPad = 8;
constexpr int pair_image_ps(int n, int K) { return (2 * K + 4) * (n * (n / 2)) + kParityPad; }
constexpr int pair_image_nrm_at(int n, int K) { return (n == 4 ? 4 : 2) * pair_image_ps(n, K); }
constexpr int pair_image_d2(int n, int K) { return pair_image_nrm_at(n, K) + (K + 2) / 2; }
constexpr int kJvpMultiMaxThreads = 256;
constexpr int jvp_multi_block(int n, int m)
{
    return n == 2 ? 8 : n == 3 ? 4 : n == 4 ? (m <= 2 ? 3 : 2) : 0;
}
constexpr bool jvp_multi_default(int n, int m)
{
    return jvp_multi_block(n, m) > 0;
}
constexpr int traj_max_threads(int n)
{
    return n == 2 ? 1024 : n == 3 ? 512 : 256;
}
constexpr size_t traj_static_lds(int n, int m, bool vjp)
{
    return (size_t)(traj_max_threads(n) / 64) * (size_t)(n * n + (vjp ? n * m : 0)) * 16;
}
template <typename F>
hipError_t dispatch_nm(int n, int m, F &&f)
{
#define GRAPE_NM_CASE(N, M) \
    case N * 8 + M: return f(std::integral_constant<int, N>{}, std::integral_constant<int, M>{})
    switch (n * 8 + m) {
        GRAPE_NM_CASE(2, 1);
        GRAPE_NM_CASE(2, 2);
        GRAPE_NM_CASE(3, 1);
        GRAPE_NM_CASE(3, 2);
        GRAPE_NM_CASE(3, 3);
        GRAPE_NM_CASE(4, 1);
        GRAPE_NM_CASE(4, 2);
        GRAPE_NM_CASE(4, 3);
        GRAPE_NM_CASE(4, 4);
    default: return hipErrorInvalidValue;
    }
#undef GRAPE_NM_CASE
}
hipError_t run_observe(int n, int sandwich, const SweepParams &p, hipStream_t stream);
hipError_t run_trajectory_vjp(int n, const SweepParams &p, hipStream_t stream);
hipError_t run_trajectory_jvp(int n, const SweepParams &p, hipStream_t stream);
hipError_t run_traj_frechet(int n, bool dir, const SweepParams &p, hipStream_t stream);
constexpr int kVjpGroup = 32;
hipError_t run_running_cost(int n, const SweepParams &p, hipStream_t stream);
hipError_t launch_fom_small(int n, int sandwich, int mode, bool pair, const SweepParams &p, hipStream_t stream);

hipError_t ensure_dynamic_lds(const void *fn, size_t lds);

hipError_t launch_sweep_small(int n, int sandwich, int mode, const SweepParams &p, hipStream_t stream);
int sweep_small_max_waves(int n);
size_t sweep_small_lds_bytes(int n, int MPB, int LT, int S, int K, bool xg_in_lds);

hipError_t launch_sweep_pair(int n, int sandwich, int mode, const SweepParams &p, hipStream_t stream);
int sweep_pair_max_waves(int n);
size_t sweep_pair_lds_bytes(int n, int MPB, int LT, int S, int K, bool xg_in_lds, bool plast = false);

struct TileParams {
    const double2 *ops;
    const double *x;
    double2 *props;
    double2 *states;
    double2 *costates;
    double *member_out;
    int32_t K, N, E, n;
    int32_t pack2;
    int32_t E_members;
    int32_t E_plan;
    int32_t s_forced, variant;
    int32_t bt_in_lds;
    int32_t stage_ops;
    int32_t prop_slices;
    int32_t unitary;
    int32_t herm_states;
    int32_t split_at;
    int32_t split_expm;
    int32_t n_x;
    int32_t thin;
    int32_t herm_ctrl;
    const double2 *vecs;
    int32_t cus;
    int32_t tp_chunks, tp_S;
    int32_t tp_window;
    int32_t tp_scan;
// ... 167 lines not shown
```

### quoptimalcontrol.jl_amd/csrc/sweep_pair.hip

```cpp
#include "cmatp.hpp"
#include "grape_kernels.hpp"

#ifndef GRAPE_ABL
#define GRAPE_ABL 0
#endif
#ifndef GRAPE_PD
#define GRAPE_PD 2
#endif
#ifndef GRAPE_PLAYOUT
#define GRAPE_PLAYOUT 0
#endif
#ifndef GRAPE_PD_EARLY
#define GRAPE_PD_EARLY 2
#endif
#ifndef GRAPE_PD_EARLY_AT
#define GRAPE_PD_EARLY_AT 0
#endif
#ifndef GRAPE_MBAR
#define GRAPE_MBAR 2
#endif

namespace grape {

enum { PMODE_GENERAL = 0, PMODE_GENERAL_KEEPL = 1, PMODE_UNITARY = 2, PMODE_UNITARY_AH = 3 };
constexpr int kAhImage = 5;

template <int N>
GRAPE_DEV int gelem(int q, int r, int jl)
{
    constexpr int NC = N / 2;
    const int i = (((r / NC) ^ q) * NC) + (r % NC);
    const int j = q * NC + jl;
    return i + j * N;
}

template <int N>
GRAPE_DEV void pstore_ws(double2 *__restrict__ base, size_t stride, const PMat<N> &m, int q)
{
#pragma unroll
    for (int jl = 0; jl < N / 2; ++jl)
#pragma unroll
        for (int r = 0; r < N; ++r)
            base[(size_t)gelem<N>(q, r, jl) * stride] = make_double2(m.re[r + jl * N], m.im[r + jl * N]);
}

template <int N>
GRAPE_DEV void pstore_ws_split(double2 *__restrict__ sbase, const unsigned (&voff)[2], size_t stride, const PMat<N> &m)
{
#pragma unroll
    for (int jl = 0; jl < N / 2; ++jl)
#pragma unroll
        for (int r = 0; r < N; ++r) {
            char *row = reinterpret_cast<char *>(sbase + (size_t)((r % (N / 2)) + jl * N) * stride);
            *reinterpret_cast<double2 *>(row + voff[r / (N / 2)]) = make_double2(m.re[r + jl * N], m.im[r + jl * N]);
        }
}

template <int N>
GRAPE_DEV void pload_ws(PMat<N> &m, const double2 *__restrict__ base, size_t stride, int q)
{
#pragma unroll
    for (int jl = 0; jl < N / 2; ++jl)
#pragma unroll
        for (int r = 0; r < N; ++r) {
            const double2 v = base[(size_t)gelem<N>(q, r, jl) * stride];
            m.re[r + jl * N] = v.x;
            m.im[r + jl * N] = v.y;
        }
}

template <int N>
GRAPE_DEV void pload_lds(PMat<N> &m, const double2 *s)
{
#pragma unroll
    for (int e = 0; e < N * (N / 2); ++e) {
        const double2 v = s[e];
        m.re[e] = v.x;
        m.im[e] = v.y;
    }
}

template <int N>
GRAPE_DEV void pstore_lds(double2 *s, const PMat<N> &m)
{
#pragma unroll
    for (int e = 0; e < N * (N / 2); ++e)
        s[e] = make_double2(m.re[e], m.im[e]);
}

GRAPE_DEV void pstamp(unsigned long long *__restrict__ st, int slot)
{
    if (st) {
        const unsigned long long t = __builtin_readcyclecounter();
        if ((threadIdx.x & 63) == 0)
            st[slot] = t;
    }
}

typedef double d2v __attribute__((ext_vector_type(2)));
struct PBuf {
    d2v v[8];
};

GRAPE_DEV void pbuf_issue(PBuf &b, unsigned voff0, unsigned voff1, const double2 *sb0, const double2 *sb1, const double2 *sb4,
                          const double2 *sb5)
{
    asm volatile("global_load_dwordx4 %0, %8, %10\n\t"
                 "global_load_dwordx4 %1, %8, %11\n\t"
// ... 29 lines not shown

GRAPE_DEV void member_barrier(unsigned *cnt, unsigned target)
{
    asm volatile("s_waitcnt lgkmcnt(0)" ::: "memory");
    if ((threadIdx.x & 63) == 0)
        __hip_atomic_fetch_add(cnt, 1u, __ATOMIC_RELAXED, __HIP_MEMORY_SCOPE_WORKGROUP);
    while (__hip_atomic_load(cnt, __ATOMIC_RELAXED, __HIP_MEMORY_SCOPE_WORKGROUP) < target)
        __builtin_amdgcn_s_sleep(1);
    asm volatile("" ::: "memory");
}

GRAPE_DEV void lds_barrier()
{
    asm volatile("s_waitcnt lgkmcnt(0)" ::: "memory");
    __builtin_amdgcn_s_barrier();
    asm volatile("" ::: "memory");
}

template <int N, int SAND>
GRAPE_DEV double pfigure_of_merit(double zr, double zi)
{
    if (SAND) {
        const double inv = 1.0 / (double)N;
        const double ar = zr * inv, ai = zi * inv;
        return 1.0 - (ar * ar + ai * ai);
    }
    return zr * zr - zi * zi;
}

template <int N, int SAND>
GRAPE_DEV void pwrite_gradient(double *out, const double2 *s_bt, int K, const PMat<N> &M, double zr, double zi,
                               double gs, int p)
{
    constexpr int NE = N * (N / 2);
    PMat<N> Z;
#pragma unroll
    for (int e = 0; e < NE; ++e) {
        if (SAND) {
            Z.re[e] = M.re[e];
            Z.im[e] = M.im[e];
        } else {
            Z.re[e] = fma(M.re[e], zr, -M.im[e] * zi);
            Z.im[e] = fma(M.re[e], zi, M.im[e] * zr);
        }
    }
    double2 b0[NE], b1[NE];
#pragma unroll
    for (int e = 0; e < NE; ++e)
        b0[e] = s_bt[e];
    for (int c = 0; c < K; c += 2) {
        if (c + 1 < K) {
#pragma unroll
            for (int e = 0; e < NE; ++e)
                b1[e] = s_bt[(c + 1) * NE + e];
        }
        double re = 0.0;
#pragma unroll
        for (int e = 0; e < NE; ++e) {
            re = fma(b0[e].x, Z.re[e], re);
            re = fma(-b0[e].y, Z.im[e], re);
        }
        re += pair_swap(re);
        if (p == 0)
            out[c] = gs * re;
        if (c + 1 < K) {
            if (c + 2 < K) {
#pragma unroll
                for (int e = 0; e < NE; ++e)
                    b0[e] = s_bt[(c + 2) * NE + e];
            }
            double r1 = 0.0;
#pragma unroll
            for (int e = 0; e < NE; ++e) {
                r1 = fma(b1[e].x, Z.re[e], r1);
                r1 = fma(-b1[e].y, Z.im[e], r1);
            }
            r1 += pair_swap(r1);
            if (p == 0)
                out[c + 1] = gs * r1;
        }
    }
}

GRAPE_DEV void pwrite_gradient_antih(double *out, const double2 *s_img, int K, const PAntiH<4> &h, double gs, int p)
{
    auto dot = [&](const double2 (&w)[kAhImage]) {
        double re = w[0].x * h.di[0];
        re = fma(w[0].y, h.di[1], re);
        re = fma(w[1].x, h.ur[2], re);
        re = fma(w[1].y, h.ui[2], re);
        re = fma(w[2].x, h.ore[0], re);
        re = fma(w[2].y, h.oim[0], re);
        re = fma(w[3].x, h.ore[3], re);
        re = fma(w[3].y, h.oim[3], re);
        re = fma(w[4].x, h.ore[2], re);
        re = fma(w[4].y, h.oim[2], re);
        return re + pair_swap(re);
    };
    double2 b0[kAhImage], b1[kAhImage];
#pragma unroll
    for (int e = 0; e < kAhImage; ++e)
        b0[e] = s_img[e];
    for (int c = 0; c < K; c += 2) {
        if (c + 1 < K) {
#pragma unroll
            for (int e = 0; e < kAhImage; ++e)
                b1[e] = s_img[(c + 1) * kAhImage + e];
        }
        const double re = dot(b0);
        if (p == 0)
            out[c] = gs * re;
        if (c + 1 < K) {
            if (c + 2 < K) {
#pragma unroll
                for (int e = 0; e < kAhImage; ++e)
                    b0[e] = s_img[(c + 2) * kAhImage + e];
            }
            const double r1 = dot(b1);
            if (p == 0)
                out[c + 1] = gs * r1;
        }
    }
}

constexpr int kVecSlices = 16;

constexpr int kPairXBatch = 16, kPairImgBatch = 4;

template <int N, int SAND, int MODE, int MAXT, bool XGLDS, bool DUMPW, bool VEC, bool IMG>
GRAPE_DEV void sweep_pair_body(const double2 *__restrict__ ops_all, const double *__restrict__ x_all,
                               const double *__restrict__ wts_all, const SweepParams &p)
{
    constexpr int NN = N * N, NC = N / 2, NE = N * NC;
    constexpr int MAXW = MAXT / 64;
    constexpr bool AH = (MODE == PMODE_UNITARY_AH);
    constexpr bool UNI = (MODE == PMODE_UNITARY) || AH;
    constexpr bool KEEPL = (MODE == PMODE_GENERAL_KEEPL);
    static_assert(!AH || (N == 4 && !SAND && !DUMPW && !VEC), "the anti-Hermitian sweep serves UnitaryGate at n = 4, first-order gradient");
    constexpr bool PDASM = (GRAPE_PD == 2) && UNI && N == 4 && !DUMPW && XGLDS;
    extern __shared__ double2 s_dyn[];
    double2(*s_tot)[MAXW][NN] = reinterpret_cast<double2(*)[MAXW][NN]>(s_dyn);
    unsigned long long t_in_real = 0, t_in_cyc = 0;
    if (p.stamps) {
        t_in_real = __builtin_amdgcn_s_memrealtime();
        t_in_cyc = __builtin_readcyclecounter();
    }

    const int LT = p.LT, W = LT >> 6, CH = LT >> 1;
    const int mb = __builtin_amdgcn_readfirstlane(threadIdx.x / LT);
    const int L = threadIdx.x - mb * LT;
    const int lane = L & 63, wave = L >> 6;
    const int par = L & 1;
    const int ch = L >> 1;
    const int cw = lane >> 1;
    const int wbase_tot = mb * W;
    const int xi = blockIdx.x / p.BPX;
    const int bi = blockIdx.x - xi * p.BPX;
    int kl = bi * p.MPB + mb;
    const bool valid = kl < p.E;
    if (!valid)
        kl = p.E - 1;
    const int k = xi * p.E + kl;
    const int K = p.K, Nsl = p.N, S = p.S;
    const size_t stride = (size_t)CH;
    const int NM = 2 * K + 4;

    unsigned *s_cnt = reinterpret_cast<unsigned *>(s_dyn + 2 * MAXW * NN);
    double2 *s_ops_all = s_dyn + 2 * MAXW * NN + 4;
    const int PS = NM * NE + kParityPad;
    double2 *s_ops = s_ops_all + (size_t)mb * 2 * PS;
    const int SK = S * K;
    const size_t nrm_d2 = ((size_t)p.MPB * (K + 1) + 1) / 2;
    double *s_xg_all = XGLDS ? reinterpret_cast<double *>(s_ops_all + (size_t)p.MPB * 2 * PS + nrm_d2)
                             : p.xg_scratch + (size_t)blockIdx.x * ((size_t)p.MPB * CH * (SK + 1) + p.MPB);
    double *s_xg = s_xg_all + (size_t)mb * CH * (SK + 1);
    double *s_F = s_xg_all + (size_t)p.MPB * CH * (SK + 1);
    double2 *s_plast = reinterpret_cast<double2 *>(s_F + ((p.MPB + 1) & ~1));
    double *s_nrm = reinterpret_cast<double *>(s_ops_all + (size_t)p.MPB * 2 * PS) + (size_t)mb * (K + 1);
    const unsigned magic = p.sk_magic;
    auto chunk_of = [&](int q) { return SK == 1 ? q : (int)__umulhi((unsigned)q, magic); };
    if (threadIdx.x < 16)
        s_cnt[threadIdx.x] = 0u;
    if (p.tune & 7) {
        const int sel = p.tune & 7;
        const bool hi = sel == 1 ? (mb & 1) : sel == 2 ? (mb & 2) : sel == 3 ? (blockIdx.x & 1) : sel == 4 ? ((threadIdx.x >> 6) & 1) : false;
        if (hi)
            __builtin_amdgcn_s_setprio(2);
    }
    if constexpr (IMG) {
        const double *__restrict__ xsrc = x_all + (size_t)xi * K * Nsl;
        const int KNs = K * Nsl, REC = 2 * PS;
        const double2 *__restrict__ rec0 = p.pair_img + (size_t)kl * pair_image_d2(N, K);
        const double2 *__restrict__ rec = rec0 + (AH ? REC : 0);
        const double *__restrict__ rnrm = reinterpret_cast<const double *>(rec0 + pair_image_nrm_at(N, K));
        double v[kPairXBatch];
        d2v im[kPairImgBatch];
        const int sk1 = SK == 1 ? -1 : 0;
#pragma unroll
        for (int u = 0; u < kPairImgBatch; ++u)
            im[u] = reinterpret_cast<const d2v *>(rec)[min(u * LT + L, REC - 1)];
        const double nr = rnrm[min(L, K)];
#pragma unroll
        for (int u = 0; u < kPairXBatch; ++u)
            v[u] = xsrc[min(u * LT + L, KNs - 1)];
        __builtin_amdgcn_sched_barrier(0);
#pragma unroll
        for (int u = 0; u < kPairImgBatch; ++u)
            reinterpret_cast<d2v *>(s_ops)[min(u * LT + L, REC - 1)] = im[u];
        s_nrm[min(L, K)] = nr;
#pragma unroll
        for (int u = 0; u < kPairXBatch; ++u) {
            const int q = min(u * LT + L, KNs - 1);
            s_xg[q + (int)__umulhi((unsigned)q, magic) + (q & sk1)] = v[u];
        }
        __syncthreads();
    } else {
    {
        const double *__restrict__ xsrc = x_all + (size_t)xi * K * Nsl;
        const int KNs = K * Nsl;
        for (int q0 = 0; q0 < KNs; q0 += 8 * LT) {
            double v[8];
#pragma unroll
            for (int u = 0; u < 8; ++u) {
                const int q = q0 + u * LT + L;
                v[u] = q < KNs ? xsrc[q] : 0.0;
            }
#pragma unroll
            for (int u = 0; u < 8; ++u) {
                const int q = q0 + u * LT + L;
                if (q < KNs)
                    s_xg[q + chunk_of(q)] = v[u];
            }
        }
        const double2 *__restrict__ ops = ops_all + (size_t)kl * (K + 3) * NN;
        for (int idx = L; idx < 2 * NM * NE; idx += LT) {
            const int q = idx / (NM * NE), rem = idx - q * NM * NE;
            const int mat = rem / NE, e = rem - mat * NE;
            if (mat == 2 * K + 3 || (AH && mat > K && mat <= 2 * K))
                continue;
            const int r = e % N, jl = e / N;
            const int i = (((r / NC) ^ q) * NC) + (r % NC), j = q * NC + jl;
            int src;
            if (mat <= K)            src = mat * NN + i + j * N;
            else if (mat <= 2 * K)   src = (mat - K) * NN + j + i * N;
            else                     src = (mat - K) * NN + i + j * N;
            s_ops[(size_t)q * PS + rem] = ops[src];
        }
    }
    if constexpr (AH) {
        const double2 *__restrict__ ops = ops_all + (size_t)kl * (K + 3) * NN;
        for (int idx = L; idx < 2 * K * 2 * kAhImage; idx += LT) {
            const int q = idx / (K * 2 * kAhImage), rem = idx - q * (K * 2 * kAhImage);
            const int c = rem / (2 * kAhImage), sl = rem - c * (2 * kAhImage);
            const int P0 = q * NC, Q0 = (1 - q) * NC;
            int jj, ii;
            double wt = 1.0;
            if (sl < 2)       { jj = ii = P0 + sl; }
            else if (sl < 4)  { jj = P0 + 1; ii = P0; wt = 2.0; }
            else if (sl < 6)  { jj = P0; ii = Q0; }
            else if (sl < 8)  { jj = P0 + 1; ii = Q0 + 1; }
            else              { jj = P0 + 1; ii = Q0; wt = 2.0; }
            const double2 b1 = ops[(size_t)(1 + c) * NN + jj + ii * N], b2 = ops[(size_t)(1 + c) * NN + ii + jj * N];
            const double bsr = 0.5 * (b1.x - b2.x), bsi = 0.5 * (b1.y + b2.y);
            const double v = sl < 2 ? -bsi : ((sl & 1) ? -wt * bsi : wt * bsr);
            reinterpret_cast<double *>(s_ops + (size_t)q * PS + (size_t)(1 + K) * NE)[c * 2 * kAhImage + sl] = v;
        }
    }
    if (L < 2 * NE) {
        const double2 *__restrict__ ops = ops_all + (size_t)kl * (K + 3) * NN;
        const double2 *__restrict__ gXi = ops + (size_t)(1 + K) * NN, *__restrict__ gXt = gXi + NN;
        const int q = L / NE, e = L - q * NE;
        const int r = e % N, jl = e / N;
        const int i = (((r / NC) ^ q) * NC) + (r % NC), j = q * NC + jl;
        double sr = 0.0, si = 0.0;
        for (int kk = 0; kk < N; ++kk) {
            const double2 a = gXi[i + kk * N], b = gXt[j + kk * N];
            sr = fma(a.x, b.x, sr); sr = fma(a.y, b.y, sr);
            si = fma(a.y, b.x, si); si = fma(-a.x, b.y, si);
        }
        s_ops[(size_t)q * PS + (size_t)(2 * K + 3) * NE + e] = make_double2(sr, si);
    }
    __syncthreads();
    if (L <= K) {
        double best = 0.0;
        for (int q = 0; q < 2; ++q)
            for (int jl = 0; jl < NC; ++jl) {
                double cs = 0.0;
                for (int r = 0; r < N; ++r) {
                    const double2 v = s_ops[(size_t)q * PS + (size_t)L * NE + r + jl * N];
                    cs += fabs(v.x) + fabs(v.y);
                }
                best = fmax(best, cs);
            }
        s_nrm[L] = best;
    }
    __syncthreads();
    }
    const double2 *sA = s_ops + (size_t)par * PS;
    const double2 *sB = sA + NE;
    const double2 *sBT = sA + (size_t)(1 + K) * NE;
    const double2 *sXi = sA + (size_t)(1 + 2 * K) * NE;
    const double2 *sXt = sXi + NE;
    const double2 *sXi_o = s_ops + (size_t)(1 - par) * PS + (size_t)(1 + 2 * K) * NE;
    const double2 *sXt_o = sXi_o + NE;
    const double2 *sXX = sXt + NE, *sXX_o = sXt_o + NE;
    double *xg = s_xg + ch * (SK + 1);
    const size_t wbase = (size_t)k * S * NN * stride + ch;
    const size_t pstep = GRAPE_PLAYOUT ? (size_t)p.E * p.n_x * NN * stride : (size_t)NN * stride;
    double2 *__restrict__ Pw = p.props + (GRAPE_PLAYOUT ? (size_t)k * NN * stride + ch : wbase);
    double2 *__restrict__ Xw = p.states + wbase;
    double *__restrict__ out = p.member_out + (size_t)k * ((size_t)K * Nsl + 1);
    const int t0 = ch * S;
    const unsigned p_rowb = (unsigned)CH * 16u;
    const unsigned p_voff[2] = {(unsigned)(par * NC + par * NC * N) * p_rowb + (unsigned)ch * 16u,
                                (unsigned)((1 - par) * NC + par * NC * N) * p_rowb + (unsigned)ch * 16u};
    double2 *__restrict__ const p_Pk = p.props + (size_t)k * (GRAPE_PLAYOUT ? 1 : S) * NN * stride;
    unsigned long long *__restrict__ st =
        p.stamps ? p.stamps + ((size_t)k * W + __builtin_amdgcn_readfirstlane(wave)) * kStampSlots : nullptr;
    if (st && lane == 0) {
        st[8] = t_in_real;
        st[9] = t_in_cyc;
        st[5] = __builtin_amdgcn_s_memrealtime();
    }
    pstamp(st, 0);

    PMat<N> Q, Q2;
    auto build = [&](int j, PMat<N> &G) -> double {
        double nb = s_nrm[0];
        double2 b0[NE], b1[NE];
#pragma unroll
        for (int e = 0; e < NE; ++e)
            b0[e] = sB[e];
        if (p.variant != 0)
            pload_lds(G, sA);
        for (int c = 0; c < K; c += 2) {
            const int c1 = min(c + 1, K - 1), c2 = min(c + 2, K - 1);
            const double x0 = xg[j * K + c];
            const double x1 = (c + 1 < K) ? xg[j * K + c1] : 0.0;
            nb = fma(fabs(x0), s_nrm[1 + c], nb);
            nb = fma(fabs(x1), s_nrm[1 + c1], nb);
#pragma unroll
            for (int e = 0; e < NE; ++e)
                b1[e] = sB[c1 * NE + e];
            if (c == 0 && p.variant == 0) {
#pragma unroll
                for (int e = 0; e < NE; ++e) {
                    G.re[e] = b0[e].x * x0;
                    G.im[e] = b0[e].y * x0;
                }
            } else {
#pragma unroll
                for (int e = 0; e < NE; ++e) {
                    G.re[e] = fma(b0[e].x, x0, G.re[e]);
                    G.im[e] = fma(b0[e].y, x0, G.im[e]);
                }
            }
#pragma unroll
            for (int e = 0; e < NE; ++e)
                b0[e] = sB[c2 * NE + e];
#pragma unroll
            for (int e = 0; e < NE; ++e) {
                G.re[e] = fma(b1[e].x, x1, G.re[e]);
                G.im[e] = fma(b1[e].y, x1, G.im[e]);
            }
        }
        if (p.variant == 0) {
#pragma unroll
            for (int e = 0; e < NE; ++e) {
                const double2 a = sA[e];
                G.re[e] += a.x;
                G.im[e] += a.y;
            }
        }
        return nb;
    };
    auto slice = [&](int j, PMat<N> &G, double nb, const PMat<N> &Qin, PMat<N> &Qout, bool first) {
        PMat<N> P, Ppar;
        __builtin_amdgcn_sched_barrier(0);
        if (GRAPE_ABL & 32) P = G; else
        pexpm_t8<N, UNI>(P, G, p.s_forced, nb);
        __builtin_amdgcn_sched_barrier(0);
        if (!(GRAPE_ABL & 2))
        pstore_ws_split(p_Pk + (size_t)j * pstep, p_voff, stride, P);
        if (UNI && XGLDS && p.plast_lds && j == S - 1) {
#pragma unroll
            for (int e = 0; e < NE; ++e)
                s_plast[e * blockDim.x + threadIdx.x] = make_double2(P.re[e], P.im[e]);
        }
        PMat<N> R;
        if (GRAPE_ABL & 4) { R = Qin; R.re[0] += P.re[1]; } else if (first) {
            R = P;
        } else {
            fetch_partner(Ppar, P);
            pmul(R, P, Ppar, Qin);
        }
        Qout = R;
        if (MODE == PMODE_GENERAL && !VEC)
            pstore_ws(Xw + (size_t)j * NN * stride, stride, Qout, par);
        __builtin_amdgcn_sched_barrier(0);
    };
    if (__all(t0 + S <= Nsl)) {
        PMat<N> G;
        pset_identity(Q);
        int j = 0;
        for (; j + 1 < S; j += 2) {
            double nb = build(j, G);
            slice(j, G, nb, Q, Q2, j == 0);
            nb = build(j + 1, G);
            slice(j + 1, G, nb, Q2, Q, false);
        }
        if (j < S) {
            const double nb = build(j, G);
            slice(j, G, nb, Q, Q2, j == 0);
            Q = Q2;
        }
    } else {
        PMat<N> G;
        pset_identity(Q);
        for (int j = 0; j < S; ++j) {
            if (t0 + j < Nsl) {
                const double nb = build(j, G);
                slice(j, G, nb, Q, Q2, j == 0);
                Q = Q2;
            }
        }
    }

    pstamp(st, 1);
#if GRAPE_PD == 2
    PBuf bA, bB;
    constexpr int PD_EARLY = (SAND && GRAPE_PD_EARLY > 1) ? 1 : GRAPE_PD_EARLY;
    auto pd_issue = [&](PBuf &b, int jj) {
        const double2 *s0 = p_Pk + (size_t)max(jj, 0) * pstep;
        pbuf_issue(b, p_voff[0], p_voff[1], s0, s0 + CH, s0 + 4 * CH, s0 + 5 * CH);
    };
    auto pd_early = [&]() {
        if constexpr (PDASM && PD_EARLY >= 1) {
            const int jm0 = (XGLDS && p.plast_lds) ? S - 2 : S - 1;
            pd_issue(bA, jm0);
            if (PD_EARLY >= 2)
                pd_issue(bB, jm0 - 1);
        }
    };
    if (W == 1 || GRAPE_PD_EARLY_AT == 0)
        pd_early();
#endif
    PMat<N> Xs, Le;
    PAntiH<N> Ah;
    double zr = 0.0, zi = 0.0;
    {
        PMat<N> inc = Q, oth, tmp, ipar;
        for (int d = 1; d < 32; d <<= 1) {
            pshfl_up(oth, inc, 2 * d);
            if (cw >= d) {
                fetch_partner(ipar, inc);
                pmul(tmp, inc, ipar, oth);
                inc = tmp;
            }
        }
        if (!UNI) {
            pshfl_up(oth, inc, 2);
            if (cw == 0)
                pset_identity(oth);
        }
        if (W > 1) {
            if (cw == 31)
                pstore_lds(&s_tot[0][wbase_tot + wave][par * NE], inc);
            if (GRAPE_MBAR == 1 && UNI)
                member_barrier(&s_cnt[mb], (unsigned)W);
            else if (GRAPE_MBAR == 2 && UNI)
                lds_barrier();
            else
                __syncthreads();
#if GRAPE_PD == 2
            if (GRAPE_PD_EARLY_AT == 1)
                pd_early();
#endif
            if (wave > 0) {
                PMat<N> pre, wt, wtp;
                pload_lds(pre, &s_tot[0][wbase_tot][par * NE]);
                for (int w = 1; w < wave; ++w) {
                    pload_lds(wt, &s_tot[0][wbase_tot + w][par * NE]);
                    pload_lds(wtp, &s_tot[0][wbase_tot + w][(1 - par) * NE]);
                    pmul(tmp, wt, wtp, pre);
                    pre = tmp;
                }
                if (UNI) {
                    fetch_partner(ipar, inc);
                    pmul(tmp, inc, ipar, pre);
                    inc = tmp;
                } else {
                    fetch_partner(ipar, oth);
                    pmul(tmp, oth, ipar, pre);
                    oth = tmp;
                }
            }
        }
        if (UNI) {
            if (ch == CH - 1)
                pstore_lds(&s_tot[1][wbase_tot][par * NE], inc);
            if (GRAPE_MBAR == 1)
                member_barrier(&s_cnt[mb], (unsigned)(W > 1 ? 2 * W : W));
            else if (GRAPE_MBAR == 2)
                lds_barrier();
            else
                __syncthreads();
            PMat<N> T, C0, xi_m, xi_o;
            pload_lds(T, &s_tot[1][wbase_tot][par * NE]);
            if (SAND) {
                PMat<N> Em, Ep;
                {
                    PMat<N> xt_m, xt_o;
                    pload_lds(xt_m, sXt);
                    pload_lds(xt_o, sXt_o);
                    pmul(tmp, xt_m, xt_o, T);
                }
                {
                    PMat<N> Tp;
                    pload_lds(Tp, &s_tot[1][wbase_tot][(1 - par) * NE]);
                    pmul_ah_b(Em, T, Tp, tmp);
                }
// ... 40 lines not shown
                pmul_a_bh(Xs, tmp, tp, oth, ipar);
            } else {
                pmul(Xs, oth, ipar, xi_m);
            }
        }
    }
    if (!UNI) {
        PMat<N> inc = Q, oth, tmp, opar;
        for (int d = 1; d < 32; d <<= 1) {
            pshfl_down(oth, inc, 2 * d);
            if (cw + d < 32) {
                fetch_partner(opar, oth);
                pmul(tmp, oth, opar, inc);
                inc = tmp;
            }
        }
        pshfl_down(oth, inc, 2);
        if (cw == 31)
            pset_identity(oth);
        if (W > 1) {
            if (cw == 0)
                pstore_lds(&s_tot[1][wbase_tot + wave][par * NE], inc);
            __syncthreads();
            if (wave + 1 < W) {
                PMat<N> post, wt, wtp;
                pload_lds(post, &s_tot[1][wbase_tot + wave + 1][par * NE]);
                for (int w = wave + 2; w < W; ++w) {
                    pload_lds(wt, &s_tot[1][wbase_tot + w][par * NE]);
                    pload_lds(wtp, &s_tot[1][wbase_tot + w][(1 - par) * NE]);
                    pmul(tmp, wt, wtp, post);
                    post = tmp;
                }
                PMat<N> pp;
                fetch_partner(pp, post);
                pmul(tmp, post, pp, oth);
                oth = tmp;
            }
        }
        PMat<N> xt_m;
        pload_lds(xt_m, sXt);
        fetch_partner(opar, oth);
        if (SAND) {
            pmul_ah_b(tmp, oth, opar, xt_m);
            PMat<N> tp;
            fetch_partner(tp, tmp);
            pmul(Le, tmp, tp, oth);
        } else {
            pmul_ah_b(Le, oth, opar, xt_m);
        }
    }

    const double gs = SAND ? -1.0 : (p.variant == 0 ? -2.0 : 2.0);

    if (UNI) {
        pstamp(st, 2);
        pstamp(st, 3);
        PMat<N> M = Xs, Mp, tmp, PA, PB, Pp;
        auto products_ah = [&](const PMat<N> &P) {
            if constexpr (AH) {
                fetch_partner(Pp, P);
                pah_own(M, Ah);
                pah_partner(Mp, Ah);
                pmul_antih_a(tmp, M, Mp, P);
                pmul_ah_b_antih(Ah, P, Pp, tmp);
            }
        };
        auto step = [&](int j, const PMat<N> &P) {
            const int t = t0 + j;
            if ((GRAPE_ABL & 64) && t < Nsl) {
#pragma unroll
                for (int e = 0; e < NE; ++e) {
                    M.re[e] += P.re[e];
                    M.im[e] += P.im[e];
                }
                double acc = 0.0;
#pragma unroll
                for (int e = 0; e < NE; ++e)
                    acc += M.re[e] + M.im[e];
                if (par == 0) xg[j * K] = acc;
            } else
            if constexpr (AH) {
                if (t < Nsl) {
                    products_ah(P);
                    pwrite_gradient_antih(xg + j * K, sBT, K, Ah, gs, par);
                    if (t == Nsl - 1 && par == 0)
                        s_F[mb] = pfigure_of_merit<N, SAND>(zr, zi);
                }
            } else
            if (t < Nsl) {
                fetch_partner(Pp, P);
                fetch_partner(Mp, M);
                pmul(tmp, M, Mp, P);
                pmul_ah_b(M, P, Pp, tmp);
                if (!SAND) {
                    double tr_r, tr_i;
                    ptrace(tr_r, tr_i, M);
                    zr = tr_r;
                    zi = -tr_i;
                }
                if (DUMPW) {
                    fetch_partner(Mp, M);
                    pmul_a_bh(tmp, M, Mp, P, Pp);
                    pstore_ws(Xw + (size_t)j * NN * stride, stride, tmp, par);
                    if (t == Nsl - 1 && par == 0) {
                        p.zphi[2 * (size_t)k] = zr;
                        p.zphi[2 * (size_t)k + 1] = -zi;
                    }
                }
                if (GRAPE_ABL & 16) { if (par == 0) xg[j * K] = M.re[0] + zr; } else
                pwrite_gradient<N, SAND>(xg + j * K, sBT, K, M, zr, zi, gs, par);
                if (t == Nsl - 1 && par == 0)
                    s_F[mb] = pfigure_of_merit<N, SAND>(zr, zi);
            }
        };
        if (XGLDS && p.plast_lds) {
#pragma unroll
            for (int e = 0; e < NE; ++e) {
                const double2 v = s_plast[e * blockDim.x + threadIdx.x];
                PA.re[e] = v.x;
                PA.im[e] = v.y;
            }
        } else if (!PDASM) {
            pload_ws(PA, Pw + (size_t)(S - 1) * pstep, stride, par);
        }
        int j = S - 1;
#if GRAPE_PD == 1
        static_assert(!AH, "the anti-Hermitian sweep is written for GRAPE_PD 0 and 2");
        auto products = [&](int jj, const PMat<N> &P) {
            if (t0 + jj < Nsl) {
                fetch_partner(Pp, P);
                fetch_partner(Mp, M);
                pmul(tmp, M, Mp, P);
                pmul_ah_b(M, P, Pp, tmp);
            }
        };
        auto gradient = [&](int jj) {
            const int t = t0 + jj;
            if (t < Nsl) {
                if (!SAND) {
                    double tr_r, tr_i;
                    ptrace(tr_r, tr_i, M);
                    zr = tr_r;
                    zi = -tr_i;
                }
                pwrite_gradient<N, SAND>(xg + jj * K, sBT, K, M, zr, zi, gs, par);
                if (t == Nsl - 1 && par == 0)
                    s_F[mb] = pfigure_of_merit<N, SAND>(zr, zi);
            }
        };
        if (DUMPW) {
            for (; j >= 0; --j) {
                if (j < S - 1 || !(XGLDS && p.plast_lds))
                    pload_ws(PA, Pw + (size_t)j * pstep, stride, par);
                step(j, PA);
            }
        } else {
            pload_ws(PB, Pw + (size_t)max(j - 1, 0) * NN * stride, stride, par);
            for (; j >= 1; j -= 2) {
                products(j, PA);
                pload_ws(PA, Pw + (size_t)max(j - 2, 0) * NN * stride, stride, par);
                gradient(j);
                products(j - 1, PB);
                pload_ws(PB, Pw + (size_t)max(j - 3, 0) * NN * stride, stride, par);
                gradient(j - 1);
            }
            if (j == 0) {
                products(0, PA);
                gradient(0);
            }
        }
#elif GRAPE_PD == 2
        if constexpr (PDASM) {
            auto products = [&](int jj, const PMat<N> &P) {
                if (t0 + jj < Nsl) {
                    if constexpr (AH) {
                        products_ah(P);
                    } else {
                        fetch_partner(Pp, P);
                        fetch_partner(Mp, M);
                        pmul(tmp, M, Mp, P);
                        pmul_ah_b(M, P, Pp, tmp);
                    }
                }
            };
            auto gradient = [&](int jj) {
                const int t = t0 + jj;
                if constexpr (AH) {
                    if (t < Nsl) {
                        pwrite_gradient_antih(xg + jj * K, sBT, K, Ah, gs, par);
                        if (t == Nsl - 1 && par == 0)
                            s_F[mb] = pfigure_of_merit<N, SAND>(zr, zi);
                    }
                } else
                if (t < Nsl) {
                    if (!SAND) {
                        double tr_r, tr_i;
                        ptrace(tr_r, tr_i, M);
                        zr = tr_r;
                        zi = -tr_i;
                    }
                    pwrite_gradient<N, SAND>(xg + jj * K, sBT, K, M, zr, zi, gs, par);
                    if (t == Nsl - 1 && par == 0)
                        s_F[mb] = pfigure_of_merit<N, SAND>(zr, zi);
                }
            };
            const bool plast = XGLDS && p.plast_lds;
            const int jm = plast ? S - 2 : S - 1;
            if (PD_EARLY >= 1) {
                pbuf_wait<0>(bA);
                if (PD_EARLY >= 2)
                    pbuf_wait<0>(bB);
            } else {
                asm volatile("s_waitcnt vmcnt(0)" ::: "memory");
                pd_issue(bA, jm);
            }
            if (PD_EARLY < 2)
                pd_issue(bB, jm - 1);
            if (plast) {
                products(j, PA);
                gradient(j);
            }
            for (j = jm; j >= 1; j -= 2) {
                pbuf_wait<8>(bA);
                pbuf_to_mat(PA, bA);
                products(j, PA);
                pd_issue(bA, j - 2);
                gradient(j);
                pbuf_wait<8>(bB);
                pbuf_to_mat(PB, bB);
                products(j - 1, PB);
                pd_issue(bB, j - 3);
                gradient(j - 1);
            }
            if (j == 0) {
                pbuf_wait<8>(bA);
                pbuf_to_mat(PA, bA);
                products(0, PA);
                gradient(0);
            }
            pbuf_wait<0>(bA);
            pbuf_wait<0>(bB);
        } else {
            for (; j >= 1; j -= 2) {
                pload_ws(PB, Pw + (size_t)(j - 1) * pstep, stride, par);
                step(j, PA);
                if (j >= 2)
                    pload_ws(PA, Pw + (size_t)(j - 2) * pstep, stride, par);
                step(j - 1, PB);
            }
            if (j == 0)
                step(0, PA);
        }
#else
        for (; j >= 1; j -= 2) {
            if (!(GRAPE_ABL & 8)) pload_ws(PB, Pw + (size_t)(j - 1) * pstep, stride, par);
            step(j, PA);
            if (j >= 2 && !(GRAPE_ABL & 8))
                pload_ws(PA, Pw + (size_t)(j - 2) * pstep, stride, par);
            step(j - 1, PB);
        }
        if (j == 0)
            step(0, PA);
#endif
    } else {
        pstamp(st, 2);
        if (KEEPL) {
            PMat<N> X = Xs, Po, Pp, Xp, tmp;
            for (int j = 0; j < S; ++j) {
                const int t = t0 + j;
                if (t < Nsl) {
                    pstore_ws(Xw + (size_t)j * NN * stride, stride, X, par);
                    if (j + 1 < S) {
                        pload_ws(Po, Pw + (size_t)j * pstep, stride, par);
                        pload_ws(Pp, Pw + (size_t)j * pstep, stride, 1 - par);
                        if (SAND) {
                            fetch_partner(Xp, X);
                            pmul_a_bh(tmp, X, Xp, Po, Pp);
                            pmul(X, Po, Pp, tmp);
                        } else {
                            pmul(tmp, Po, Pp, X);
                            X = tmp;
                        }
                    }
                }
            }
        }

        pstamp(st, 3);
        if constexpr (VEC) {
            static_assert(N == 4 && !SAND && MODE == PMODE_GENERAL, "the vector sweep serves left multiplication at n = 4");
            constexpr int SV = kVecSlices;
            double xr[SV + 1][2], xi_[SV + 1][2];
            {
                const double a2 = pair_swap(Xs.re[2]), b2 = pair_swap(Xs.im[2]), a3 = pair_swap(Xs.re[3]), b3 = pair_swap(Xs.im[3]);
                xr[0][0] = par ? a2 : Xs.re[0];
                xi_[0][0] = par ? b2 : Xs.im[0];
                xr[0][1] = par ? a3 : Xs.re[1];
                xi_[0][1] = par ? b3 : Xs.im[1];
            }
            double wr[2], wi[2];
            {
                const double a2 = pair_swap(Le.re[2]), b2 = pair_swap(Le.im[2]), a3 = pair_swap(Le.re[3]), b3 = pair_swap(Le.im[3]);
                wr[0] = par ? a2 : Le.re[0];
// ... 66 lines not shown
                        const double2 *bc = sB + (size_t)c * NE;
                        double ar = 0.0, ai = 0.0;
#pragma unroll
                        for (int jl = 0; jl < 2; ++jl) {
                            double ur = 0.0, ui = 0.0;
#pragma unroll
                            for (int r = 0; r < 4; ++r) {
                                const double2 b = bc[r + 4 * jl];
                                ur = fma(lr[r], b.x, ur);
                                ur = fma(li[r], b.y, ur);
                                ui = fma(lr[r], b.y, ui);
                                ui = fma(-li[r], b.x, ui);
                            }
                            ar = fma(ur, xr[j][jl], ar);
                            ar = fma(-ui, xi_[j][jl], ar);
                            ai = fma(ur, xi_[j][jl], ai);
                            ai = fma(ui, xr[j][jl], ai);
                        }
                        ar += pair_swap(ar);
                        ai += pair_swap(ai);
                        if (par == 0)
                            xg[j * K + c] = gs * fma(zr_, ar, -zi_ * ai);
                    }
                    if (t == Nsl - 1 && par == 0)
                        s_F[mb] = pfigure_of_merit<N, SAND>(zr_, zi_);
                }
            }
        } else {
        PMat<N> Lc = Le, Po, Pp, X, Xp, M, tmp, Lp;
        for (int j = S - 1; j >= 0; --j) {
            const int t = t0 + j;
            if (t < Nsl) {
                pload_ws(Po, Pw + (size_t)j * pstep, stride, par);
                pload_ws(Pp, Pw + (size_t)j * pstep, stride, 1 - par);
                if (SAND) {
                    fetch_partner(Lp, Lc);
                    pmul(tmp, Lc, Lp, Po);
                    pmul_ah_b(Lc, Po, Pp, tmp);
                } else {
                    pmul_ah_b(tmp, Po, Pp, Lc);
                    Lc = tmp;
                }
                if (KEEPL) {
                    pload_ws(X, Xw + (size_t)j * NN * stride, stride, par);
                } else if (j > 0) {
                    PMat<N> Qo, Qp;
                    pload_ws(Qo, Xw + (size_t)(j - 1) * NN * stride, stride, par);
                    pload_ws(Qp, Xw + (size_t)(j - 1) * NN * stride, stride, 1 - par);
                    if (SAND) {
                        pmul(tmp, Qo, Qp, Xs);
                        PMat<N> tp;
                        fetch_partner(tp, tmp);
                        pmul_a_bh(X, tmp, tp, Qo, Qp);
                    } else {
                        pmul(X, Qo, Qp, Xs);
                    }
                } else {
                    X = Xs;
                }
                if (KEEPL)
                    pstore_ws(p.costates + wbase + (size_t)j * NN * stride, stride, Lc, par);
                double zr, zi;
                ptrace_ah_b(zr, zi, X, Lc);
                fetch_partner(Xp, X);
                fetch_partner(Lp, Lc);
                pmul_a_bh(M, X, Xp, Lc, Lp);
                if (SAND) {
                    pmul_ah_b(tmp, Lc, Lp, X);
#pragma unroll
                    for (int e = 0; e < NE; ++e) {
                        M.re[e] -= tmp.re[e];
                        M.im[e] -= tmp.im[e];
                    }
                }
                pwrite_gradient<N, SAND>(xg + j * K, sBT, K, M, zr, zi, gs, par);
                if (t == Nsl - 1 && par == 0)
                    s_F[mb] = pfigure_of_merit<N, SAND>(zr, zi);
            }
        }
        }
    }
    __syncthreads();
    const int KN = K * Nsl;
    if (p.member_out && valid) {
        for (int q = L; q < KN; q += LT)
            out[q] = s_xg[q + chunk_of(q)];
        if (L == 0)
            out[KN] = s_F[mb];
    }
    {
        const int nmem = min(p.MPB, p.E - bi * p.MPB);
        const double *__restrict__ wb = wts_all + (size_t)bi * p.MPB;
        double *__restrict__ bout = p.block_out + (size_t)blockIdx.x * (KN + 1);
        const int mstride = CH * (SK + 1);
        for (int q = threadIdx.x; q <= KN; q += blockDim.x) {
            const int off = q + chunk_of(q);
            double acc = 0.0;
            for (int m = 0; m < nmem; ++m) {
                const double v = (q < KN) ? s_xg_all[m * mstride + off] : s_F[m];
                acc = fma(v, wb[m], acc);
            }
            bout[q] = acc;
            if (p.direct_dst)
                p.direct_dst[q] = acc;
        }
    }
    if (p.direct_flag) {
        __threadfence_system();
        __syncthreads();
        if (threadIdx.x == 0)
            __hip_atomic_store(p.direct_flag, p.direct_seq, __ATOMIC_RELEASE, __HIP_MEMORY_SCOPE_SYSTEM);
    }
    pstamp(st, 4);
    if (st && lane == 0) {
        st[6] = __builtin_amdgcn_s_memrealtime();
        st[7] = ((unsigned long long)__builtin_amdgcn_s_getreg(20 | (31 << 11)) << 32) |
                (unsigned)__builtin_amdgcn_s_getreg(4 | (31 << 11));
    }
}

template <int N, int SAND, int MODE, int MAXT, bool XGLDS, bool DUMPW = false, bool VEC = false>
__global__ __launch_bounds__(MAXT) void sweep_pair_kernel(const double2 *__restrict__ ops_all,
                                                          const double *__restrict__ x_all,
                                                          const double *__restrict__ wts_all,
                                                          const SweepParams p)
{
    sweep_pair_body<N, SAND, MODE, MAXT, XGLDS, DUMPW, VEC, XGLDS>(ops_all, x_all, wts_all, p);
}

template <int N, int SAND, int MODE, int MAXT, bool XGLDS, bool DUMPW = false, bool VEC = false>
__global__ __launch_bounds__(MAXT) void sweep_pair_build_kernel(const double2 *__restrict__ ops_all,
                                                                const double *__restrict__ x_all,
                                                                const double *__restrict__ wts_all,
                                                                const SweepParams p)
{
    sweep_pair_body<N, SAND, MODE, MAXT, XGLDS, DUMPW, VEC, false>(ops_all, x_all, wts_all, p);
}

template <int N>
__global__ __launch_bounds__(64) void pair_image_kernel(const double2 *__restrict__ ops_all, double2 *__restrict__ img_all,
                                                        int K, int E)
{
    constexpr int NN = N * N, NC = N / 2, NE = N * NC;
    constexpr bool AH = (N == 4);
    const int kl = blockIdx.x, L = threadIdx.x, LT = blockDim.x;
    if (kl >= E)
        return;
    const int NM = 2 * K + 4, PS = pair_image_ps(N, K), REC = 2 * PS;
    const double2 *__restrict__ ops = ops_all + (size_t)kl * (K + 3) * NN;
    double2 *__restrict__ rec = img_all + (size_t)kl * pair_image_d2(N, K);
    auto ah_weight = [&](int q, int c, int sl) {
        const int P0 = q * NC, Q0 = (1 - q) * NC;
        int jj, ii;
        double wt = 1.0;
        if (sl < 2)       { jj = ii = P0 + sl; }
        else if (sl < 4)  { jj = P0 + 1; ii = P0; wt = 2.0; }
        else if (sl < 6)  { jj = P0; ii = Q0; }
        else if (sl < 8)  { jj = P0 + 1; ii = Q0 + 1; }
        else              { jj = P0 + 1; ii = Q0; wt = 2.0; }
        const double2 b1 = ops[(size_t)(1 + c) * NN + jj + ii * N], b2 = ops[(size_t)(1 + c) * NN + ii + jj * N];
        const double bsr = 0.5 * (b1.x - b2.x), bsi = 0.5 * (b1.y + b2.y);
        const double v = sl < 2 ? -bsi : ((sl & 1) ? -wt * bsi : wt * bsr);
        return v;
    };
    for (int idx = L; idx < REC; idx += LT) {
        const int q = idx / PS, rem = idx - q * PS;
        const int mat = rem / NE, e = rem - mat * NE;
        double2 val = make_double2(0.0, 0.0), val_ah = val;
        if (mat == 2 * K + 3) {
            const double2 *__restrict__ gXi = ops + (size_t)(1 + K) * NN, *__restrict__ gXt = gXi + NN;
            const int r = e % N, jl = e / N;
            const int i = (((r / NC) ^ q) * NC) + (r % NC), j = q * NC + jl;
            double sr = 0.0, si = 0.0;
            for (int kk = 0; kk < N; ++kk) {
                const double2 a = gXi[i + kk * N], b = gXt[j + kk * N];
                sr = fma(a.x, b.x, sr); sr = fma(a.y, b.y, sr);
                si = fma(a.y, b.x, si); si = fma(-a.x, b.y, si);
            }
            val = val_ah = make_double2(sr, si);
        } else if (mat < NM) {
            const int r = e % N, jl = e / N;
            const int i = (((r / NC) ^ q) * NC) + (r % NC), j = q * NC + jl;
            int src;
            if (mat <= K)            src = mat * NN + i + j * N;
            else if (mat <= 2 * K)   src = (mat - K) * NN + j + i * N;
            else                     src = (mat - K) * NN + i + j * N;
            val = val_ah = ops[src];
            if (AH && mat > K && mat <= 2 * K) {
                const int d0 = 2 * (rem - (1 + K) * NE);
                val_ah = make_double2(0.0, 0.0);
                if (d0 < K * 2 * kAhImage) {
                    const int c = d0 / (2 * kAhImage), sl = d0 - c * (2 * kAhImage);
                    val_ah = make_double2(ah_weight(q, c, sl), ah_weight(q, c, sl + 1));
                }
            }
        }
        rec[idx] = val;
        if (AH)
            rec[REC + idx] = val_ah;
    }
    if (L <= K) {
        double best = 0.0;
        for (int q = 0; q < 2; ++q)
            for (int jl = 0; jl < NC; ++jl) {
                double cs = 0.0;
                for (int r = 0; r < N; ++r) {
                    const double2 v = ops[(size_t)L * NN + gelem<N>(q, r, jl)];
                    cs += fabs(v.x) + fabs(v.y);
                }
                best = fmax(best, cs);
            }
        reinterpret_cast<double *>(rec + pair_image_nrm_at(N, K))[L] = best;
    }
}

static hipError_t run_pair_image(int n, const SweepParams &p, hipStream_t stream)
{
    if (!p.pair_img || p.E < 1)
        return hipErrorInvalidValue;
    if (n == 2)
        GRAPE_LAUNCH_AS("pair_image_kernel", pair_image_kernel<2>, dim3(p.E), dim3(64), 0, stream, p.ops, p.pair_img, p.K, p.E);
    else if (n == 4)
        GRAPE_LAUNCH_AS("pair_image_kernel", pair_image_kernel<4>, dim3(p.E), dim3(64), 0, stream, p.ops, p.pair_img, p.K, p.E);
    else
        return hipErrorInvalidValue;
    return hipGetLastError();
}

template <int N>
struct PairTraits;
template <> struct PairTraits<2> { static constexpr int MAXT = 1024; };
template <> struct PairTraits<4> { static constexpr int MAXT = 512; };

int sweep_pair_max_waves(int n)
{
    switch (n) {
    case 2: return PairTraits<2>::MAXT / 64;
    case 4: return PairTraits<4>::MAXT / 64;
    default: return 0;
    }
}

size_t sweep_pair_lds_bytes(int n, int MPB, int LT, int S, int K, bool xg_in_lds, bool plast)
{
    const int maxt = n == 2 ? PairTraits<2>::MAXT : PairTraits<4>::MAXT;
    size_t b = sizeof(double2) * (2 * (size_t)(maxt / 64) * n * n + 4);
    b += sizeof(double2) * ((size_t)MPB * 2 * ((2 * K + 4) * (n * (n / 2)) + kParityPad) + ((size_t)MPB * (K + 1) + 1) / 2);
    if (xg_in_lds)
        b += sizeof(double) * ((size_t)MPB * (LT / 2) * ((size_t)S * K + 1) + ((MPB + 1) & ~1));
    if (plast)
        b += sizeof(double2) * (size_t)MPB * LT * (n * (n / 2));
    return b;
}

template <int N, int SAND, int MODE, int MAXT, bool XGLDS, bool DUMPW, bool VEC>
static auto pair_build_kernel()
{
    if constexpr (XGLDS)
        return sweep_pair_build_kernel<N, SAND, MODE, MAXT, XGLDS, DUMPW, VEC>;
    else
        return sweep_pair_kernel<N, SAND, MODE, MAXT, XGLDS, DUMPW, VEC>;
}

template <int N, int SAND, int MODE, bool XGLDS>
static hipError_t plaunch_one(const SweepParams &p0, hipStream_t stream)
{
    constexpr int MAXT = PairTraits<N>::MAXT;
    SweepParams p = p0;
    const dim3 grid(p.BPX * p.n_x), block(p.LT * p.MPB);
    size_t lds = sweep_pair_lds_bytes(N, p.MPB, p.LT, p.S, p.K, XGLDS);
    if (lds > 160 * 1024)
        return hipErrorInvalidConfiguration;
    p.plast_lds = 0;
    {
        static const int tune_env = [] { const char *e = getenv("GRAPE_PAIR_TUNE"); return e ? atoi(e) : 0; }();
        p.tune = tune_env;
    }
    if ((MODE == PMODE_UNITARY || MODE == PMODE_UNITARY_AH) && XGLDS && p.S > 1) {
        const size_t with = sweep_pair_lds_bytes(N, p.MPB, p.LT, p.S, p.K, true, true);
        if (with <= 160 * 1024) {
            p.plast_lds = 1;
            lds = with;
        }
    }
    const bool copy = XGLDS && p.pair_img && (long long)p.K * p.N <= (long long)kPairXBatch * p.LT &&
                      2 * pair_image_ps(N, p.K) <= kPairImgBatch * p.LT;
    auto go = [&](auto kern_copy, auto kern_build, const char *name) -> hipError_t {
        auto kern = copy ? kern_copy : kern_build;
        if (lds > 64 * 1024) {
            hipError_t e = ensure_dynamic_lds((const void *)kern, lds);
            if (e != hipSuccess)
                return e;
        }
        GRAPE_LAUNCH_AS(name, kern, grid, block, lds, stream, p.ops, p.x, p.wts, p);
        return hipGetLastError();
    };
    if constexpr (MODE == PMODE_UNITARY && SAND == 0) {
        if (p.dump_w1) {
            return go(sweep_pair_kernel<N, SAND, MODE, MAXT, XGLDS, true>, pair_build_kernel<N, SAND, MODE, MAXT, XGLDS, true, false>(), "sweep_pair_kernel");
        }
    }
    if (p.dump_w1)
        return hipErrorInvalidConfiguration;
    if constexpr (N == 4 && SAND == 0 && MODE == PMODE_GENERAL && XGLDS) {
        if (p.vec && p.S <= kVecSlices) {
            return go(sweep_pair_kernel<N, SAND, MODE, MAXT, XGLDS, false, true>, pair_build_kernel<N, SAND, MODE, MAXT, XGLDS, false, true>(), "sweep_pair_vec_kernel");
        }
    }
    return go(sweep_pair_kernel<N, SAND, MODE, MAXT, XGLDS>, pair_build_kernel<N, SAND, MODE, MAXT, XGLDS, false, false>(), "sweep_pair_kernel");
}

template <int N, int SAND>
static hipError_t plaunch_ns(int mode, const SweepParams &p, hipStream_t stream)
{
    constexpr int MAXT = PairTraits<N>::MAXT;
    if (p.MPB < 1 || p.LT * p.MPB > MAXT || (p.LT & 63) || (long long)p.S * (p.LT / 2) < p.N)
        return hipErrorInvalidConfiguration;
    const bool lds = p.xg_scratch == nullptr;
    switch (mode) {
    case PMODE_GENERAL:
        return lds ? plaunch_one<N, SAND, PMODE_GENERAL, true>(p, stream) : plaunch_one<N, SAND, PMODE_GENERAL, false>(p, stream);
    case PMODE_GENERAL_KEEPL:
        return lds ? plaunch_one<N, SAND, PMODE_GENERAL_KEEPL, true>(p, stream)
                   : plaunch_one<N, SAND, PMODE_GENERAL_KEEPL, false>(p, stream);
    case PMODE_UNITARY:
        return lds ? plaunch_one<N, SAND, PMODE_UNITARY, true>(p, stream) : plaunch_one<N, SAND, PMODE_UNITARY, false>(p, stream);
    case PMODE_UNITARY_AH:
        if constexpr (N == 4 && SAND == 0)
            return lds ? plaunch_one<N, SAND, PMODE_UNITARY_AH, true>(p, stream)
                       : plaunch_one<N, SAND, PMODE_UNITARY_AH, false>(p, stream);
        return hipErrorInvalidConfiguration;
    default:
        return hipErrorInvalidValue;
    }
}

hipError_t launch_sweep_pair(int n, int sandwich, int mode, const SweepParams &p, hipStream_t stream)
{
    if (p.img_only)
        return run_pair_image(n, p, stream);
    if (p.fom_only)
        return launch_fom_small(n, sandwich, mode, true, p, stream);
    if (p.rc_only)
        return run_running_cost(n, p, stream);
    if (p.obs_only)
        return run_observe(n, sandwich, p, stream);
    if (p.vjp_only)
        return run_trajectory_vjp(n, p, stream);
    if (p.jvp_only)
        return run_trajectory_jvp(n, p, stream);
    switch (n * 2 + (sandwich ? 1 : 0)) {
    case 4: return plaunch_ns<2, 0>(mode, p, stream);
    case 5: return plaunch_ns<2, 1>(mode, p, stream);
    case 8: return plaunch_ns<4, 0>(mode, p, stream);
    case 9: return plaunch_ns<4, 1>(mode, p, stream);
    default: return hipErrorInvalidValue;
    }
}

}
```

Measured before the change: 13100 gradient-evals/s.

## Keep last propagators on chip, skip their global store, compact anti-Hermitian image

Lets the pair sweep kernel hold up to two propagators per chunk in LDS instead of one. When the host owns the control upload and no trajectory, observable or exact-gradient consumer needs them, it also skips writing those propagators to global memory. Any later trajectory or controls request replays the sweep to materialize the skipped propagators. The anti-Hermitian LDS image is shrunk to a compact layout, and in the two-on-chip mode the gradient scratch is moved into the plast area. This trades more LDS and extra host-side bookkeeping for less global write traffic.

```diff
diff --git a/quoptimalcontrol.jl_amd/csrc/grape_api.cpp b/quoptimalcontrol.jl_amd/csrc/grape_api.cpp
--- a/quoptimalcontrol.jl_amd/csrc/grape_api.cpp
+++ b/quoptimalcontrol.jl_amd/csrc/grape_api.cpp
@@ -210,6 +210,10 @@
     bool risk_evaluated = false;
     std::vector<double> h_wts;
     bool pair_ah_env = true;
+    int pair_onchip_env = 2;
+    bool debug_env = false;
+    bool x_owned = false, props_skipped = false, traj_latch = false;
+    int owned_nx = 1;
     bool mf_publish = true;
     unsigned long long seq = 0;
     std::string kernel_log;
@@ -809,6 +813,9 @@
         c->mf_publish = !env_off("GRAPE_MF_PUBLISH");
         c->pair_ah_env = !env_off("GRAPE_PAIR_AH");
         c->pair_image_env = !env_off("GRAPE_PAIR_IMAGE");
+        const char *oc = std::getenv("GRAPE_PAIR_ONCHIP");
+        if (oc && oc[0] >= '0' && oc[0] <= '2' && !oc[1]) c->pair_onchip_env = oc[0] - '0';
+        c->debug_env = std::getenv("GRAPE_DEBUG") != nullptr;
     }
     {
         const char *xu = std::getenv("GRAPE_X_UPLOAD");
@@ -1267,6 +1274,7 @@
 }
 
 static int wait_stream(grape_ctx *c, hipStream_t stream);
+static int materialize_props(grape_ctx *c);
 
 static int risk_check_weights(const grape_ctx *c, const double *wts, const char *who)
 {
@@ -1410,6 +1418,7 @@
     grape_ctx *lead = lead_of(c);
     HIP_TRY(c, hipSetDevice(lead->device));
     if (int rc = order_behind_device_call(c, lead)) return rc;
+    if (int rc = materialize_props(c)) return rc;
     std::memcpy(lead->h_stage, theta, sizeof(double) * KP(c));
     const grape::BasisOp op = basis_op(c, false, 1);
     grape::DoneSignal d;
@@ -2060,6 +2069,7 @@
     c->h_wts.assign(wts, wts + E);
     c->ops_set = true;
     c->evaluated = false;
+    c->props_skipped = false;
     c->risk_evaluated = false;
     return GRAPE_OK;
 }
@@ -2191,6 +2201,8 @@
     p.s_forced = c->cfg.expm_squarings;
     p.variant = c->cfg.variant;
     p.dt = c->cfg.duration / c->cfg.n_slices;
+    p.onchip_want = c->pair_onchip_env;
+    p.onchip_debug = c->debug_env ? 1 : 0;
     return p;
 }
 
@@ -2479,6 +2491,9 @@
     }
     const bool exact = c->cfg.gradient == GRAPE_GRADIENT_EXACT;
     if (exact) p.member_out = nullptr;
+    p.onchip_nostore = (c->x_owned && c->pair_onchip_env >= 1 && !c->traj_latch && c->family == 0 && c->pair && c->unitary && c->cfg.n == 4 &&
+                        !rc_on && !c->obs_on && !c->vjp_on && !c->jvp_on && !exact && !c->exact_w1) ? 1 : 0;
+    c->props_skipped = p.onchip_nostore != 0;
     const bool direct = c->family == 0 && c->NB == 1 && n_x == 1 && !exact && c->direct_publish && !done.probe_out &&
                         !done.stage_base && !pen_active(c) && !rc_on && !risk;
     const bool fold = !done.stage_base && tile_folds_reduce(c, n_x);
@@ -2783,7 +2798,29 @@
         if (s->mf_publish) done.mflags = s->d_h_flag + 8;
         target = s->d_fg;
     }
-    return enqueue_eval(s, d_x, target, s->stream, n_x, done);
+    s->x_owned = true;
+    s->owned_nx = n_x;
+    const int rc = enqueue_eval(s, d_x, target, s->stream, n_x, done);
+    s->x_owned = false;
+    return rc;
+}
+
+static int materialize_props(grape_ctx *c)
+{
+    if (c->is_group) {
+        for (grape_ctx *s : c->sub)
+            if (int rc = materialize_props(s)) return fail(c, rc, s->err);
+        return GRAPE_OK;
+    }
+    if (!c->props_skipped) return GRAPE_OK;
+    const bool latch = c->traj_latch;
+    c->traj_latch = true;
+    const std::string log = c->kernel_log;
+    int rc = shard_issue(c, c->owned_nx, c->d_fg, false);
+    if (rc == GRAPE_OK) rc = wait_stream(c, c->stream);
+    c->kernel_log = log;
+    c->traj_latch = latch;
+    return rc;
 }
 
 static int shard_enqueue_host(grape_ctx *s, const double *x, int n_x, double *target, bool signal)
@@ -3695,6 +3732,7 @@
         HIP_TRY(c, hipMalloc((void **)&c->d_fom_rows, sizeof(double) * (size_t)c->NB * c->B));
     }
     const bool param = pulse_map(c);
+    if (int rc = materialize_props(c)) return rc;
     if (param)
         std::memcpy(c->h_stage, x, sizeof(double) * KP(c) * n_x);
     else
@@ -4422,6 +4460,7 @@
         int local = 0;
         grape_ctx *s = owner_of(c, member, &local);
         const int rc = grape_get_trajectory(s, local, props, states, costates);
+        for (grape_ctx *o : c->sub) o->traj_latch = true;
         return rc ? group_fail(c, s, rc) : GRAPE_OK;
     }
     if (chunked(c))
@@ -4442,6 +4481,8 @@
                     "context with GRAPE_FLAG_KEEP_COSTATES");
     HIP_TRY(c, hipSetDevice(c->device));
     HIP_TRY(c, hipDeviceSynchronize());
+    if (int rc = materialize_props(c)) return rc;
+    c->traj_latch = true;
     const int n = c->cfg.n;
     const size_t nn = (size_t)n * n, N = c->cfg.n_slices, K = c->cfg.n_controls;
     std::vector<cplx> P(N * nn);
diff --git a/quoptimalcontrol.jl_amd/csrc/grape_kernels.hpp b/quoptimalcontrol.jl_amd/csrc/grape_kernels.hpp
--- a/quoptimalcontrol.jl_amd/csrc/grape_kernels.hpp
+++ b/quoptimalcontrol.jl_amd/csrc/grape_kernels.hpp
@@ -147,9 +147,15 @@
     int64_t jvp_dir_xdot, jvp_dir_ydot, jvp_dir_xf, jvp_dir_w;
     double2 *pair_img;
     int32_t img_only;
+    int32_t onchip_want;
+    int32_t onchip;
+    int32_t onchip_nostore;
+    int32_t onchip_debug;
 };
 constexpr int kParityPad = 8;
+constexpr int kAhImage = 5;
 constexpr int pair_image_ps(int n, int K) { return (2 * K + 4) * (n * (n / 2)) + kParityPad; }
+constexpr int pair_image_psa(int K) { return (1 + K) * 8 + kAhImage * K + 8 + ((8 - (13 * K + 16)) & 15); }
 constexpr int pair_image_nrm_at(int n, int K) { return (n == 4 ? 4 : 2) * pair_image_ps(n, K); }
 constexpr int pair_image_d2(int n, int K) { return pair_image_nrm_at(n, K) + (K + 2) / 2; }
 constexpr int kJvpMultiMaxThreads = 256;
diff --git a/quoptimalcontrol.jl_amd/csrc/sweep_pair.hip b/quoptimalcontrol.jl_amd/csrc/sweep_pair.hip
--- a/quoptimalcontrol.jl_amd/csrc/sweep_pair.hip
+++ b/quoptimalcontrol.jl_amd/csrc/sweep_pair.hip
@@ -1,5 +1,8 @@
 #include "cmatp.hpp"
 #include "grape_kernels.hpp"
+#include <atomic>
+#include <cstdio>
+#include <cstdlib>
 
 #ifndef GRAPE_ABL
 #define GRAPE_ABL 0
@@ -23,7 +26,6 @@
 namespace grape {
 
 enum { PMODE_GENERAL = 0, PMODE_GENERAL_KEEPL = 1, PMODE_UNITARY = 2, PMODE_UNITARY_AH = 3 };
-constexpr int kAhImage = 5;
 
 template <int N>
 GRAPE_DEV int gelem(int q, int r, int jl)
@@ -219,8 +221,9 @@
     }
 }
 
-GRAPE_DEV void pwrite_gradient_antih(double *out, const double2 *s_img, int K, const PAntiH<4> &h, double gs, int p)
-{
+GRAPE_DEV void pwrite_gradient_antih(double *g, int gq, int w0, const double2 *s_img, int K, const PAntiH<4> &h, double gs, int p)
+{
+    auto at = [&](int w) -> double & { return g[(w >> 2) * gq + (w & 3)]; };
     auto dot = [&](const double2 (&w)[kAhImage]) {
         double re = w[0].x * h.di[0];
         re = fma(w[0].y, h.di[1], re);
@@ -246,7 +249,7 @@
         }
         const double re = dot(b0);
         if (p == 0)
-            out[c] = gs * re;
+            at(w0 + c) = gs * re;
         if (c + 1 < K) {
             if (c + 2 < K) {
 #pragma unroll
@@ -255,7 +258,7 @@
             }
             const double r1 = dot(b1);
             if (p == 0)
-                out[c + 1] = gs * r1;
+                at(w0 + c + 1) = gs * r1;
         }
     }
 }
@@ -304,15 +307,18 @@
 
     unsigned *s_cnt = reinterpret_cast<unsigned *>(s_dyn + 2 * MAXW * NN);
     double2 *s_ops_all = s_dyn + 2 * MAXW * NN + 4;
-    const int PS = NM * NE + kParityPad;
+    const int PS = AH ? pair_image_psa(K) : NM * NE + kParityPad;
+    const int XXat = AH ? (1 + K) * NE + kAhImage * K : (2 * K + 3) * NE;
     double2 *s_ops = s_ops_all + (size_t)mb * 2 * PS;
     const int SK = S * K;
     const size_t nrm_d2 = ((size_t)p.MPB * (K + 1) + 1) / 2;
+    const bool oc2 = AH && XGLDS && p.onchip == 2;
     double *s_xg_all = XGLDS ? reinterpret_cast<double *>(s_ops_all + (size_t)p.MPB * 2 * PS + nrm_d2)
                              : p.xg_scratch + (size_t)blockIdx.x * ((size_t)p.MPB * CH * (SK + 1) + p.MPB);
-    double *s_xg = s_xg_all + (size_t)mb * CH * (SK + 1);
-    double *s_F = s_xg_all + (size_t)p.MPB * CH * (SK + 1);
+    double *s_xg = s_xg_all + (oc2 ? (size_t)0 : (size_t)mb * CH * (SK + 1));
+    double *s_F = s_xg_all + (size_t)(oc2 ? 1 : p.MPB) * CH * (SK + 1);
     double2 *s_plast = reinterpret_cast<double2 *>(s_F + ((p.MPB + 1) & ~1));
+    double2 *s_plast2 = s_plast + (size_t)NE * blockDim.x;
     double *s_nrm = reinterpret_cast<double *>(s_ops_all + (size_t)p.MPB * 2 * PS) + (size_t)mb * (K + 1);
     const unsigned magic = p.sk_magic;
     auto chunk_of = [&](int q) { return SK == 1 ? q : (int)__umulhi((unsigned)q, magic); };
@@ -328,18 +334,19 @@
         const double *__restrict__ xsrc = x_all + (size_t)xi * K * Nsl;
         const int KNs = K * Nsl, REC = 2 * PS;
         const double2 *__restrict__ rec0 = p.pair_img + (size_t)kl * pair_image_d2(N, K);
-        const double2 *__restrict__ rec = rec0 + (AH ? REC : 0);
+        const double2 *__restrict__ rec = rec0 + (AH ? 2 * pair_image_ps(N, K) : 0);
         const double *__restrict__ rnrm = reinterpret_cast<const double *>(rec0 + pair_image_nrm_at(N, K));
         double v[kPairXBatch];
         d2v im[kPairImgBatch];
         const int sk1 = SK == 1 ? -1 : 0;
+        const int XL = oc2 ? (int)blockDim.x : LT, xl = oc2 ? (int)threadIdx.x : L;
 #pragma unroll
         for (int u = 0; u < kPairImgBatch; ++u)
             im[u] = reinterpret_cast<const d2v *>(rec)[min(u * LT + L, REC - 1)];
         const double nr = rnrm[min(L, K)];
 #pragma unroll
         for (int u = 0; u < kPairXBatch; ++u)
-            v[u] = xsrc[min(u * LT + L, KNs - 1)];
+            v[u] = xsrc[min(u * XL + xl, KNs - 1)];
         __builtin_amdgcn_sched_barrier(0);
 #pragma unroll
         for (int u = 0; u < kPairImgBatch; ++u)
@@ -347,7 +354,7 @@
         s_nrm[min(L, K)] = nr;
 #pragma unroll
         for (int u = 0; u < kPairXBatch; ++u) {
-            const int q = min(u * LT + L, KNs - 1);
+            const int q = min(u * XL + xl, KNs - 1);
             s_xg[q + (int)__umulhi((unsigned)q, magic) + (q & sk1)] = v[u];
         }
         __syncthreads();
@@ -355,25 +362,27 @@
     {
         const double *__restrict__ xsrc = x_all + (size_t)xi * K * Nsl;
         const int KNs = K * Nsl;
-        for (int q0 = 0; q0 < KNs; q0 += 8 * LT) {
+        const int XL = oc2 ? (int)blockDim.x : LT, xl = oc2 ? (int)threadIdx.x : L;
+        for (int q0 = 0; q0 < KNs; q0 += 8 * XL) {
             double v[8];
 #pragma unroll
             for (int u = 0; u < 8; ++u) {
-                const int q = q0 + u * LT + L;
+                const int q = q0 + u * XL + xl;
                 v[u] = q < KNs ? xsrc[q] : 0.0;
             }
 #pragma unroll
             for (int u = 0; u < 8; ++u) {
-                const int q = q0 + u * LT + L;
+                const int q = q0 + u * XL + xl;
                 if (q < KNs)
                     s_xg[q + chunk_of(q)] = v[u];
             }
         }
         const double2 *__restrict__ ops = ops_all + (size_t)kl * (K + 3) * NN;
-        for (int idx = L; idx < 2 * NM * NE; idx += LT) {
-            const int q = idx / (NM * NE), rem = idx - q * NM * NE;
+        const int NMb = AH ? 1 + K : NM;
+        for (int idx = L; idx < 2 * NMb * NE; idx += LT) {
+            const int q = idx / (NMb * NE), rem = idx - q * NMb * NE;
             const int mat = rem / NE, e = rem - mat * NE;
-            if (mat == 2 * K + 3 || (AH && mat > K && mat <= 2 * K))
+            if (mat == 2 * K + 3)
                 continue;
             const int r = e % N, jl = e / N;
             const int i = (((r / NC) ^ q) * NC) + (r % NC), j = q * NC + jl;
@@ -415,7 +424,7 @@
             sr = fma(a.x, b.x, sr); sr = fma(a.y, b.y, sr);
             si = fma(a.y, b.x, si); si = fma(-a.x, b.y, si);
         }
-        s_ops[(size_t)q * PS + (size_t)(2 * K + 3) * NE + e] = make_double2(sr, si);
+        s_ops[(size_t)q * PS + XXat + e] = make_double2(sr, si);
     }
     __syncthreads();
     if (L <= K) {
@@ -440,8 +449,10 @@
     const double2 *sXt = sXi + NE;
     const double2 *sXi_o = s_ops + (size_t)(1 - par) * PS + (size_t)(1 + 2 * K) * NE;
     const double2 *sXt_o = sXi_o + NE;
-    const double2 *sXX = sXt + NE, *sXX_o = sXt_o + NE;
+    const double2 *sXX = sA + XXat, *sXX_o = s_ops + (size_t)(1 - par) * PS + XXat;
     double *xg = s_xg + ch * (SK + 1);
+    double *const g_at = oc2 ? reinterpret_cast<double *>(s_plast) + 2 * mb * LT + 4 * ch : xg;
+    const int g_q = oc2 ? 2 * (int)blockDim.x : 4;
     const size_t wbase = (size_t)k * S * NN * stride + ch;
     const size_t pstep = GRAPE_PLAYOUT ? (size_t)p.E * p.n_x * NN * stride : (size_t)NN * stride;
     double2 *__restrict__ Pw = p.props + (GRAPE_PLAYOUT ? (size_t)k * NN * stride + ch : wbase);
@@ -517,12 +528,23 @@
         if (GRAPE_ABL & 32) P = G; else
         pexpm_t8<N, UNI>(P, G, p.s_forced, nb);
         __builtin_amdgcn_sched_barrier(0);
+        const bool keep1 = UNI && XGLDS && p.plast_lds && j >= S - 1, keep2 = oc2 && j >= S - 2 && j < S - 1;
         if (!(GRAPE_ABL & 2))
+        if (__builtin_expect(!((keep1 || keep2) && p.onchip_nostore), 1))
         pstore_ws_split(p_Pk + (size_t)j * pstep, p_voff, stride, P);
-        if (UNI && XGLDS && p.plast_lds && j == S - 1) {
+        if (__builtin_expect(keep1, 1)) {
+            unsigned T = threadIdx.x;
+            asm volatile("" : "+v"(T));
 #pragma unroll
             for (int e = 0; e < NE; ++e)
-                s_plast[e * blockDim.x + threadIdx.x] = make_double2(P.re[e], P.im[e]);
+                s_plast[e * blockDim.x + T] = make_double2(P.re[e], P.im[e]);
+        }
+        if (__builtin_expect(keep2, 1)) {
+            unsigned T = threadIdx.x;
+            asm volatile("" : "+v"(T));
+#pragma unroll
+            for (int e = 0; e < NE; ++e)
+                s_plast2[e * blockDim.x + T] = make_double2(P.re[e], P.im[e]);
         }
         PMat<N> R;
         if (GRAPE_ABL & 4) { R = Qin; R.re[0] += P.re[1]; } else if (first) {
@@ -573,7 +595,7 @@
     };
     auto pd_early = [&]() {
         if constexpr (PDASM && PD_EARLY >= 1) {
-            const int jm0 = (XGLDS && p.plast_lds) ? S - 2 : S - 1;
+            const int jm0 = S - 1 - (XGLDS ? p.onchip : 0);
             pd_issue(bA, jm0);
             if (PD_EARLY >= 2)
                 pd_issue(bB, jm0 - 1);
@@ -780,7 +802,7 @@
             if constexpr (AH) {
                 if (t < Nsl) {
                     products_ah(P);
-                    pwrite_gradient_antih(xg + j * K, sBT, K, Ah, gs, par);
+                    pwrite_gradient_antih(g_at, g_q, j * K, sBT, K, Ah, gs, par);
                     if (t == Nsl - 1 && par == 0)
                         s_F[mb] = pfigure_of_merit<N, SAND>(zr, zi);
                 }
@@ -885,7 +907,7 @@
                 const int t = t0 + jj;
                 if constexpr (AH) {
                     if (t < Nsl) {
-                        pwrite_gradient_antih(xg + jj * K, sBT, K, Ah, gs, par);
+                        pwrite_gradient_antih(g_at, g_q, jj * K, sBT, K, Ah, gs, par);
                         if (t == Nsl - 1 && par == 0)
                             s_F[mb] = pfigure_of_merit<N, SAND>(zr, zi);
                     }
@@ -902,8 +924,8 @@
                         s_F[mb] = pfigure_of_merit<N, SAND>(zr, zi);
                 }
             };
-            const bool plast = XGLDS && p.plast_lds;
-            const int jm = plast ? S - 2 : S - 1;
+            const int nlds = XGLDS ? p.onchip : 0;
+            const int jm = S - 1 - nlds;
             if (PD_EARLY >= 1) {
                 pbuf_wait<0>(bA);
                 if (PD_EARLY >= 2)
@@ -914,9 +936,20 @@
             }
             if (PD_EARLY < 2)
                 pd_issue(bB, jm - 1);
-            if (plast) {
-                products(j, PA);
-                gradient(j);
+#pragma nounroll
+            for (int r = 0; r < nlds; ++r) {
+                if constexpr (AH) {
+                    if (r) {
+#pragma unroll
+                        for (int e = 0; e < NE; ++e) {
+                            const double2 v = s_plast2[e * blockDim.x + threadIdx.x];
+                            PA.re[e] = v.x;
+                            PA.im[e] = v.y;
+                        }
+                    }
+                }
+                products(j - r, PA);
+                gradient(j - r);
             }
             for (j = jm; j >= 1; j -= 2) {
                 pbuf_wait<8>(bA);
@@ -1149,9 +1182,17 @@
     }
     __syncthreads();
     const int KN = K * Nsl;
+    auto g_of = [&](int m, int q) -> double {
+        const int cq = chunk_of(q);
+        if (oc2) {
+            const int w = q - cq * SK;
+            return reinterpret_cast<const double *>(s_plast)[(w >> 2) * g_q + 2 * m * LT + 4 * cq + (w & 3)];
+        }
+        return s_xg_all[m * (CH * (SK + 1)) + q + cq];
+    };
     if (p.member_out && valid) {
         for (int q = L; q < KN; q += LT)
-            out[q] = s_xg[q + chunk_of(q)];
+            out[q] = g_of(mb, q);
         if (L == 0)
             out[KN] = s_F[mb];
     }
@@ -1159,12 +1200,10 @@
         const int nmem = min(p.MPB, p.E - bi * p.MPB);
         const double *__restrict__ wb = wts_all + (size_t)bi * p.MPB;
         double *__restrict__ bout = p.block_out + (size_t)blockIdx.x * (KN + 1);
-        const int mstride = CH * (SK + 1);
         for (int q = threadIdx.x; q <= KN; q += blockDim.x) {
-            const int off = q + chunk_of(q);
             double acc = 0.0;
             for (int m = 0; m < nmem; ++m) {
-                const double v = (q < KN) ? s_xg_all[m * mstride + off] : s_F[m];
+                const double v = (q < KN) ? g_of(m, q) : s_F[m];
                 acc = fma(v, wb[m], acc);
             }
             bout[q] = acc;
@@ -1233,7 +1272,7 @@
     for (int idx = L; idx < REC; idx += LT) {
         const int q = idx / PS, rem = idx - q * PS;
         const int mat = rem / NE, e = rem - mat * NE;
-        double2 val = make_double2(0.0, 0.0), val_ah = val;
+        double2 val = make_double2(0.0, 0.0);
         if (mat == 2 * K + 3) {
             const double2 *__restrict__ gXi = ops + (size_t)(1 + K) * NN, *__restrict__ gXt = gXi + NN;
             const int r = e % N, jl = e / N;
@@ -1244,7 +1283,7 @@
                 sr = fma(a.x, b.x, sr); sr = fma(a.y, b.y, sr);
                 si = fma(a.y, b.x, si); si = fma(-a.x, b.y, si);
             }
-            val = val_ah = make_double2(sr, si);
+            val = make_double2(sr, si);
         } else if (mat < NM) {
             const int r = e % N, jl = e / N;
             const int i = (((r / NC) ^ q) * NC) + (r % NC), j = q * NC + jl;
@@ -1252,19 +1291,39 @@
             if (mat <= K)            src = mat * NN + i + j * N;
             else if (mat <= 2 * K)   src = (mat - K) * NN + j + i * N;
             else                     src = (mat - K) * NN + i + j * N;
-            val = val_ah = ops[src];
-            if (AH && mat > K && mat <= 2 * K) {
-                const int d0 = 2 * (rem - (1 + K) * NE);
-                val_ah = make_double2(0.0, 0.0);
-                if (d0 < K * 2 * kAhImage) {
-                    const int c = d0 / (2 * kAhImage), sl = d0 - c * (2 * kAhImage);
-                    val_ah = make_double2(ah_weight(q, c, sl), ah_weight(q, c, sl + 1));
-                }
-            }
+            val = ops[src];
         }
         rec[idx] = val;
-        if (AH)
-            rec[REC + idx] = val_ah;
+    }
+    for (int idx = L; AH && idx < REC; idx += LT) {
+        const int PSA = pair_image_psa(K), q = idx / PSA, rem = idx - q * PSA;
+        const int w_at = (1 + K) * NE, xx_at = w_at + kAhImage * K;
+        double2 val = make_double2(0.0, 0.0);
+        if (q >= 2) {
+            ;
+        } else if (rem < w_at) {
+            const int mat = rem / NE, e = rem - mat * NE;
+            const int r = e % N, jl = e / N;
+            const int i = (((r / NC) ^ q) * NC) + (r % NC), j = q * NC + jl;
+            val = ops[mat * NN + i + j * N];
+        } else if (rem < xx_at) {
+            const int d0 = 2 * (rem - w_at);
+            const int c = d0 / (2 * kAhImage), sl = d0 - c * (2 * kAhImage);
+            val = make_double2(ah_weight(q, c, sl), ah_weight(q, c, sl + 1));
+        } else if (rem < xx_at + NE) {
+            const double2 *__restrict__ gXi = ops + (size_t)(1 + K) * NN, *__restrict__ gXt = gXi + NN;
+            const int e = rem - xx_at;
+            const int r = e % N, jl = e / N;
+            const int i = (((r / NC) ^ q) * NC) + (r % NC), j = q * NC + jl;
+            double sr = 0.0, si = 0.0;
+            for (int kk = 0; kk < N; ++kk) {
+                const double2 a = gXi[i + kk * N], b = gXt[j + kk * N];
+                sr = fma(a.x, b.x, sr); sr = fma(a.y, b.y, sr);
+                si = fma(a.y, b.x, si); si = fma(-a.x, b.y, si);
+            }
+            val = make_double2(sr, si);
+        }
+        rec[REC + idx] = val;
     }
     if (L <= K) {
         double best = 0.0;
@@ -1308,16 +1367,20 @@
     }
 }
 
-size_t sweep_pair_lds_bytes(int n, int MPB, int LT, int S, int K, bool xg_in_lds, bool plast)
+static size_t pair_lds_bytes(int n, int MPB, int LT, int S, int K, bool xg_in_lds, int onchip, bool ah)
 {
     const int maxt = n == 2 ? PairTraits<2>::MAXT : PairTraits<4>::MAXT;
     size_t b = sizeof(double2) * (2 * (size_t)(maxt / 64) * n * n + 4);
-    b += sizeof(double2) * ((size_t)MPB * 2 * ((2 * K + 4) * (n * (n / 2)) + kParityPad) + ((size_t)MPB * (K + 1) + 1) / 2);
+    b += sizeof(double2) * ((size_t)MPB * 2 * (ah ? pair_image_psa(K) : pair_image_ps(n, K)) + ((size_t)MPB * (K + 1) + 1) / 2);
     if (xg_in_lds)
-        b += sizeof(double) * ((size_t)MPB * (LT / 2) * ((size_t)S * K + 1) + ((MPB + 1) & ~1));
-    if (plast)
-        b += sizeof(double2) * (size_t)MPB * LT * (n * (n / 2));
+        b += sizeof(double) * ((size_t)(onchip == 2 ? 1 : MPB) * (LT / 2) * ((size_t)S * K + 1) + ((MPB + 1) & ~1));
+    b += sizeof(double2) * (size_t)onchip * MPB * LT * (n * (n / 2));
     return b;
+}
+
+size_t sweep_pair_lds_bytes(int n, int MPB, int LT, int S, int K, bool xg_in_lds, bool plast)
+{
+    return pair_lds_bytes(n, MPB, LT, S, K, xg_in_lds, plast ? 1 : 0, false);
 }
 
 template <int N, int SAND, int MODE, int MAXT, bool XGLDS, bool DUMPW, bool VEC>
@@ -1335,23 +1398,38 @@
     constexpr int MAXT = PairTraits<N>::MAXT;
     SweepParams p = p0;
     const dim3 grid(p.BPX * p.n_x), block(p.LT * p.MPB);
-    size_t lds = sweep_pair_lds_bytes(N, p.MPB, p.LT, p.S, p.K, XGLDS);
+    constexpr bool AH = MODE == PMODE_UNITARY_AH;
+    size_t lds = pair_lds_bytes(N, p.MPB, p.LT, p.S, p.K, XGLDS, 0, AH);
     if (lds > 160 * 1024)
         return hipErrorInvalidConfiguration;
     p.plast_lds = 0;
+    p.onchip = 0;
     {
         static const int tune_env = [] { const char *e = getenv("GRAPE_PAIR_TUNE"); return e ? atoi(e) : 0; }();
         p.tune = tune_env;
     }
-    if ((MODE == PMODE_UNITARY || MODE == PMODE_UNITARY_AH) && XGLDS && p.S > 1) {
-        const size_t with = sweep_pair_lds_bytes(N, p.MPB, p.LT, p.S, p.K, true, true);
-        if (with <= 160 * 1024) {
-            p.plast_lds = 1;
-            lds = with;
-        }
-    }
-    const bool copy = XGLDS && p.pair_img && (long long)p.K * p.N <= (long long)kPairXBatch * p.LT &&
-                      2 * pair_image_ps(N, p.K) <= kPairImgBatch * p.LT;
+    if ((MODE == PMODE_UNITARY || AH) && XGLDS && p.S > 1) {
+        const bool two = AH && N == 4 && GRAPE_PD == 2 && p.onchip_want >= 2 && p.S >= 3 && p.S * p.K <= 32;
+        for (int oc = two ? 2 : 1; oc >= 1 && !p.onchip; --oc) {
+            const size_t with = pair_lds_bytes(N, p.MPB, p.LT, p.S, p.K, true, oc, AH);
+            if (with <= 160 * 1024) {
+                p.plast_lds = 1;
+                p.onchip = oc;
+                lds = with;
+            }
+        }
+    }
+    if (!(p.onchip > 0 && p.onchip_want >= 1 && N == 4 && !p.dump_w1))
+        p.onchip_nostore = 0;
+    if (p.onchip_debug) {
+        static std::atomic<long long> told{-1};
+        const long long key = ((long long)lds * 4 + p.onchip) * 8 + p.onchip_want * 2 + p.onchip_nostore;
+        if (told.exchange(key) != key)
+            fprintf(stderr, "[grape] sweep_pair: %d propagator(s) per chunk on chip%s, %zu B of LDS (GRAPE_PAIR_ONCHIP=%d)\n",
+                    p.onchip, p.onchip_nostore ? ", not stored" : "", lds, p.onchip_want);
+    }
+    const bool copy = XGLDS && p.pair_img && (long long)p.K * p.N <= (long long)kPairXBatch * p.LT * (p.onchip == 2 ? p.MPB : 1) &&
+                      2 * (AH ? pair_image_psa(p.K) : pair_image_ps(N, p.K)) <= kPairImgBatch * p.LT;
     auto go = [&](auto kern_copy, auto kern_build, const char *name) -> hipError_t {
         auto kern = copy ? kern_copy : kern_build;
         if (lds > 64 * 1024) {
```

New measurement: 13210 gradient-evals/s, median of 6. No clear change (+0.8%).
